# HengyiWang/spann3r

Measured on AMD Instinct MI355X. Metric: frames/sec/GPU (224px, 10-frame seq) + mem-bank cross-attn HBM GB/s, higher is better.
Workload: dtype bf16

## Files before the change

include/spann3r_hip.h:

```cpp
#ifndef SPANN3R_HIP_H
#define SPANN3R_HIP_H

#include <stdint.h>

#ifdef __cplusplus
extern "C" {
#endif

enum { SP3_F32 = 0, SP3_BF16 = 1 };
enum { SP3_ACT_NONE = 0, SP3_ACT_GELU = 1, SP3_ACT_RELU = 2 };
enum { SP3_EPI_PLAIN = 0, SP3_EPI_ROPE_VT = 1, SP3_EPI_PIXSHUF = 2, SP3_EPI_PARTIAL = 3 };
enum { SP3_LOAD_PLAIN = 0, SP3_LOAD_CONV3X3 = 1, SP3_LOAD_SOFTMAX = 2 };

const char* sp3_last_error(void);
int sp3_version(void);

typedef struct sp3_gemm_desc {
  const float* A;
  const float* A2;
  const void* W;
  void* C;
  const float* bias;
  const float* res1;
  const float* res2;
  int32_t M, N, K;
  int32_t batch;
  int32_t K1;
  int64_t lda, lda2, ldw, ldc, ldr1, ldr2;
  int64_t strideA, strideW, strideC;
  float alpha;
  int32_t wdtype;
  int32_t act;
  int32_t out_bf16;
  int32_t relu_in;
  int32_t loader;
  int32_t conv_H, conv_W, conv_C, conv_OH, conv_OW, conv_stride;
  int32_t epi;
  const float* rope_cos;
  const float* rope_sin;
  const int32_t* pos;
  int32_t rope_cols;
  void* vt;
  int32_t tokens;
  int32_t heads;
  int64_t vt_ld;
  int32_t ps_k, ps_H, ps_W, ps_C;
  int32_t tile;
  int32_t a_bf16;
  int32_t splitk;
  int32_t a_packed;
  const float* ln_stats;
  const float* ln_s;
  int32_t ln_nt;
  int32_t ln_C;
  float ln_eps;
  float* stats_out;
  void* c2;
  int32_t qkv_packed;
  int32_t out_packed;
  int32_t w_packed;
  int64_t sb_A2, sb_bias, sb_ln_stats, sb_ln_s, sb_stats_out, sb_c2, sb_vt;
  int64_t* trace;
  float* sm_stats_out;
  const float* sm_stats;
  int32_t sm_nt;
  float sm_thresh;
  float* sm_zout;
  int32_t f32x3;
  int32_t res_bf16;
  const int32_t* dyn_n;
} sp3_gemm_desc;
int sp3_gemm(const sp3_gemm_desc* desc_host, void* stream);
int sp3_gemm2(const sp3_gemm_desc* a, const sp3_gemm_desc* b, void* stream);
int sp3_gemm_plan(const sp3_gemm_desc* desc_host);

int sp3_layernorm(const float* x, int64_t ldx, const float* gamma, const float* beta, float eps,
                  void* out, int64_t ldo, int out_bf16, int rows, int C, void* stream);
int sp3_layernorm_packed(const float* x, int64_t ldx, const float* gamma, const float* beta, float eps,
                         void* out, int out_bf16, int rows, int C, void* stream);
int sp3_layernorm_dual(const float* x, int64_t ldx, const float* gamma, const float* beta, float eps, float* out, int64_t ldo,
                       void* out_packed_bf16, int rows, int C, int group_rows, int group_rows_pad, void* stream);
int sp3_layernorm_t(const float* x, int64_t ldx, const float* gamma, const float* beta, float eps,
                    void* out, int64_t ldo, int out_bf16, int rows, int C, void* stream);

typedef struct sp3_reduce_ln_desc {
  const float* partial;
  int64_t split_stride;
  const float* bias;
  const float* res;
  int64_t ldres;
  float* x_out;
  int64_t ldx;
  const float* g1; const float* b1; void* out1; int64_t ld1; int32_t out1_bf16;
  const float* g2; const float* b2; void* out2; int64_t ld2; int32_t out2_bf16;
  float eps;
  int32_t splits, rows, C;
  int32_t out1_packed, out2_packed;
  int32_t act;
  const float* res2;
  int64_t ldres2;
} sp3_reduce_ln_desc;
int sp3_reduce_ln(const sp3_reduce_ln_desc* desc_host, void* stream);

int sp3_rope_2d(void* tokens, int dtype, int B, int N, int H, int D, int64_t sB, int64_t sN, int64_t sH,
                const int64_t* positions, float base, float fwd, void* stream);

int sp3_attention(const void* q, int64_t sq, int64_t ldq, const void* k, int64_t sk, int64_t ldk,
                  const void* vt, int64_t vt_ld, void* out, int64_t ldo, int out_bf16,
                  int B, int heads, int Nq, int Nk, float scale, int dtype, void* stream);
int sp3_attention_ex(const void* q, int64_t sq, int64_t ldq, const void* k, int64_t sk, int64_t ldk,
                     const void* vt, int64_t vt_ld, void* out, int64_t ldo, int out_bf16, int out_packed,
                     int B, int heads, int Nq, int Nk, float scale, int dtype, void* stream);

int sp3_attention_packed(const void* qp, int q_cols, int q_col0, int npad_q, const void* kp, int k_cols, int k_col0, int npad_k,
                         const void* vtp, void* out, int64_t ldo, int out_bf16, int out_packed,
                         int B, int heads, int Nq, int Nk, float scale, int o_group, int o_group_rows, void* stream);

typedef struct sp3_attn_qproj_desc {
  const void* x_packed; int64_t x_group_stride;
  const float* ln_stats; int64_t stats_group_stride;
  const void* w_packed; int64_t w_group_stride;
  const float* ln_s; const float* bias; int64_t vec_group_stride;
  const int32_t* pos; const float* rope_cos; const float* rope_sin;
  float ln_eps; int32_t D;
  const void* kp; int32_t k_cols, k_col0, npad_k; const void* vtp;
  void* out; int64_t ldo; int32_t out_bf16, out_packed;
  int32_t B, heads, Nq, Nk; float scale; int32_t o_group, o_group_rows;
} sp3_attn_qproj_desc;
int sp3_attention_packed_qproj(const sp3_attn_qproj_desc* desc_host, void* stream);

typedef struct sp3_bank_write_desc {
  const float* feat_k;
  const float* feat_v;
  float* k_raw;
  float* v_raw;
  void* k_hat;
  void* v_hat_t;
  float* s_bank;
  float* b_bank;
  const float *gamma_k, *beta_k, *gamma_v, *beta_v, *gamma_q, *beta_q;
  float eps;
  float alpha;
  int32_t M, P, C, cap;
  int32_t wdtype;
  const int32_t* state;
} sp3_bank_write_desc;
int sp3_bank_write(const sp3_bank_write_desc* desc_host, void* stream);
int sp3_softmax_thresh(const float* S, float* P, int64_t ld, int64_t strideS, int rows, int M, int Mpad,
                       float thresh, int batch, void* P_packed, int64_t stride_packed, int packed_bf16, void* stream);
int sp3_softmax_pack(const float* S, int64_t ld, int64_t strideS, int rows, int M, float thresh, int batch, void* P_packed,
                     int64_t stride_packed, int packed_bf16, float* rowstat_ws, void* stream);
int sp3_colsum_accum(const float* P, int64_t ld, int rows, int M, float* mem_attn, void* stream);
int sp3_colsum_packed(const void* P_packed, int packed_bf16, int rows, int M, float* mem_attn, void* stream);
int sp3_colsum_softmax(const float* S, int64_t ld, int rows, int M, const float* rowz, float thresh, float* mem_attn,
                       float* mem_count, int append_P, void* stream);
int sp3_pack_stats(const float* x, int64_t ldx, int rows, int C, void* packed, int packed_bf16, float* stats, void* stream);
// ... 131 lines not shown
```

spann3r_amd/csrc/common.h:

```cpp
#pragma once
#include <hip/hip_runtime.h>
#include <stdint.h>
#include <stdio.h>
#include "../../include/spann3r_hip.h"

typedef __attribute__((ext_vector_type(8))) __bf16 bf16x8;
typedef __attribute__((ext_vector_type(4))) __bf16 bf16x4;
typedef __attribute__((ext_vector_type(2))) __bf16 bf16x2;
typedef __attribute__((ext_vector_type(4))) float f32x4;

#define SP3_WAVE 64

void sp3_set_error(const char* fmt, ...);

#define SP3_CHECK(cond, ...)                     \
  do {                                           \
    if (!(cond)) {                               \
      sp3_set_error(__VA_ARGS__);                \
      return 1;                                  \
    }                                            \
  } while (0)

#define SP3_LAUNCH_CHECK(what)                                              \
  do {                                                                      \
    hipError_t e_ = hipGetLastError();                                      \
    if (e_ != hipSuccess) {                                                 \
      sp3_set_error("%s: launch failed: %s", what, hipGetErrorString(e_));  \
      return 2;                                                             \
    }                                                                       \
  } while (0)

__device__ __forceinline__ float wave_sum(float v) {
#pragma unroll
  for (int o = 32; o > 0; o >>= 1) v += __shfl_xor(v, o);
  return v;
}
__device__ __forceinline__ float wave_max(float v) {
#pragma unroll
  for (int o = 32; o > 0; o >>= 1) v = fmaxf(v, __shfl_xor(v, o));
  return v;
}

__device__ __forceinline__ bf16x8 cvt8(const float4 a, const float4 b) {
  bf16x8 r;
  r[0] = (__bf16)a.x; r[1] = (__bf16)a.y; r[2] = (__bf16)a.z; r[3] = (__bf16)a.w;
  r[4] = (__bf16)b.x; r[5] = (__bf16)b.y; r[6] = (__bf16)b.z; r[7] = (__bf16)b.w;
  return r;
}

__device__ __forceinline__ float4 relu4(float4 v) {
  v.x = fmaxf(v.x, 0.f); v.y = fmaxf(v.y, 0.f); v.z = fmaxf(v.z, 0.f); v.w = fmaxf(v.w, 0.f);
  return v;
}

__device__ __forceinline__ float gelu_erf(float x) {
  const float a = fabsf(x);
  const float t = __builtin_amdgcn_rcpf(fmaf(0.2316419f, a, 1.0f));
  float p = fmaf(1.330274429f, t, -1.821255978f);
  p = fmaf(p, t, 1.781477937f);
  p = fmaf(p, t, -0.356563782f);
  p = fmaf(p, t, 0.319381530f);
  const float e = __builtin_amdgcn_exp2f(-0.72134752044448170368f * a * a);
  const float q = (p * t) * (e * 0.3989422804014327f);
  return fmaf(-a, q, fmaxf(x, 0.f));
}

#ifndef SP3_NO_WT_STORES
__device__ __forceinline__ void st_out(bf16x4* p, bf16x4 v) {
  __hip_atomic_store(reinterpret_cast<unsigned long long*>(p), __builtin_bit_cast(unsigned long long, v), __ATOMIC_RELAXED, __HIP_MEMORY_SCOPE_AGENT);
}
__device__ __forceinline__ void st_out(float2* p, float2 v) {
  __hip_atomic_store(reinterpret_cast<unsigned long long*>(p), __builtin_bit_cast(unsigned long long, v), __ATOMIC_RELAXED, __HIP_MEMORY_SCOPE_AGENT);
}
__device__ __forceinline__ void st_out(float4* p, float4 v) {
  const f32x4 t = {v.x, v.y, v.z, v.w};
  asm volatile("global_store_dwordx4 %0, %1, off sc1\n\ts_nop 1" ::"v"(p), "v"(t) : "memory");
}
__device__ __forceinline__ void st_out(bf16x8* p, bf16x8 v) {
  asm volatile("global_store_dwordx4 %0, %1, off sc1\n\ts_nop 1" ::"v"(p), "v"(v) : "memory");
}
#else
template <typename T> __device__ __forceinline__ void st_out(T* p, T v) { *p = v; }
#endif

__device__ __forceinline__ int64_t packed_off(int row, int k, int K, bool bf16) {
  const int lkb = bf16 ? 6 : 5, lch = bf16 ? 4 : 3;
  const int nkb = (K + (1 << lkb) - 1) >> lkb;
  const int kb = k >> lkb, kk = k & ((1 << lkb) - 1);
  const int g = kk >> lch, e = kk & ((1 << lch) - 1);
  const int h = e >> (lch - 1), eh = e & ((1 << (lch - 1)) - 1);
  return (((((int64_t)(row >> 4) * nkb + kb) * 2 + h) * 4 + g) * 16 + (row & 15)) * (1 << (lch - 1)) + eh;
}
```

spann3r_amd/csrc/gemm.hip:

```cpp
#include "common.h"
#include "gemm_sm.h"
#include <cstdlib>
#include <type_traits>

namespace {

struct GemmArgs {
  sp3_gemm_desc d;
  sp3_gemm_desc d2;
  int nb1;
  int xcd_slices;
};

template <typename TA, typename TW> struct MM;

__device__ __forceinline__ bf16x8 zero8() {
  bf16x8 z;
#pragma unroll
  for (int i = 0; i < 8; ++i) z[i] = (__bf16)0.f;
  return z;
}

__device__ __forceinline__ bf16x8 relu8(bf16x8 v) {
#pragma unroll
  for (int i = 0; i < 8; ++i) v[i] = (float)v[i] > 0.f ? v[i] : (__bf16)0.f;
  return v;
}

typedef __attribute__((ext_vector_type(4))) unsigned int u32x4;

__device__ __forceinline__ bf16x8 mask8(bf16x8 v, unsigned m) {
  u32x4 b = __builtin_bit_cast(u32x4, v);
  b &= m;
  return __builtin_bit_cast(bf16x8, b);
}
__device__ __forceinline__ float4 mask4(float4 v, unsigned m) {
  v.x = __uint_as_float(__float_as_uint(v.x) & m);
  v.y = __uint_as_float(__float_as_uint(v.y) & m);
  v.z = __uint_as_float(__float_as_uint(v.z) & m);
  v.w = __uint_as_float(__float_as_uint(v.w) & m);
  return v;
}

struct WRegB { bf16x8 v[2]; };
__device__ __forceinline__ void loadW_b(WRegB& r, const __bf16* p, int off1) {
  r.v[0] = *reinterpret_cast<const bf16x8*>(p);
  r.v[1] = *reinterpret_cast<const bf16x8*>(p + off1);
}
__device__ __forceinline__ void fixW_b(WRegB& r, unsigned m0, unsigned m1) {
  r.v[0] = mask8(r.v[0], m0);
  r.v[1] = mask8(r.v[1], m1);
}

template <> struct MM<float, __bf16> {
  static constexpr int KB = 64;
  static constexpr int CH = 16;
  struct AReg { float4 v[4]; };
  using WReg = WRegB;
  static __device__ __forceinline__ void loadA(AReg& r, const float* p, int off1) {
    const float4* q = reinterpret_cast<const float4*>(p);
    const float4* q1 = reinterpret_cast<const float4*>(p + off1);
    r.v[0] = q[0]; r.v[1] = q[1]; r.v[2] = q1[0]; r.v[3] = q1[1];
  }
  static __device__ __forceinline__ void fixA(AReg& r, unsigned m0, unsigned m1, bool relu) {
    r.v[0] = mask4(r.v[0], m0); r.v[1] = mask4(r.v[1], m0); r.v[2] = mask4(r.v[2], m1); r.v[3] = mask4(r.v[3], m1);
    if (relu) { r.v[0] = relu4(r.v[0]); r.v[1] = relu4(r.v[1]); r.v[2] = relu4(r.v[2]); r.v[3] = relu4(r.v[3]); }
  }
  static __device__ __forceinline__ void loadW(WReg& r, const __bf16* p, int off1) { loadW_b(r, p, off1); }
  static __device__ __forceinline__ void fixW(WReg& r, unsigned m0, unsigned m1) { fixW_b(r, m0, m1); }
  template <int MF, int NF>
  static __device__ __forceinline__ void mma(f32x4 (&acc)[MF][NF], const AReg (&a)[MF], const WReg (&w)[NF]) {
#pragma unroll
    for (int m = 0; m < MF; ++m) {
      const bf16x8 a0 = cvt8(a[m].v[0], a[m].v[1]);
      const bf16x8 a1 = cvt8(a[m].v[2], a[m].v[3]);
#pragma unroll
      for (int n = 0; n < NF; ++n) {
        acc[m][n] = __builtin_amdgcn_mfma_f32_16x16x32_bf16(a0, w[n].v[0], acc[m][n], 0, 0, 0);
        acc[m][n] = __builtin_amdgcn_mfma_f32_16x16x32_bf16(a1, w[n].v[1], acc[m][n], 0, 0, 0);
      }
    }
  }
  template <int MF, int NF>
  static __device__ __forceinline__ void mma_half(f32x4 (&)[MF][NF], const AReg (&)[MF], const WReg (&)[NF]) {}
};

template <> struct MM<__bf16, __bf16> {
  static constexpr int KB = 64;
  static constexpr int CH = 16;
  struct AReg { bf16x8 v[2]; };
  using WReg = WRegB;
  static __device__ __forceinline__ void loadA(AReg& r, const __bf16* p, int off1) {
    r.v[0] = *reinterpret_cast<const bf16x8*>(p);
// ... 220 lines not shown
  const TA* base[MF];
  __device__ __forceinline__ void init(const sp3_gemm_desc& d, const TA* A, int row0, int lane, int, int) {
#pragma unroll
    for (int m = 0; m < MF; ++m) {
      int r = row0 + m * 16 + (lane & 15);
      r = r < d.M ? r : d.M - 1;
      base[m] = A + (int64_t)r * d.lda;
    }
  }
  __device__ __forceinline__ const TA* ptr(const sp3_gemm_desc&, int m, int k, int, int, bool& inb) const {
    inb = true;
    return base[m] + k;
  }
};

__device__ __forceinline__ float4 smx4(float4 s, float c, float thr, int left, float& z) {
  constexpr float L2E = 1.44269504088896341f;
  float p[4] = {__builtin_amdgcn_exp2f(fmaf(s.x, L2E, c)), __builtin_amdgcn_exp2f(fmaf(s.y, L2E, c)),
                __builtin_amdgcn_exp2f(fmaf(s.z, L2E, c)), __builtin_amdgcn_exp2f(fmaf(s.w, L2E, c))};
#pragma unroll
  for (int e = 0; e < 4; ++e) {
    p[e] = (p[e] < thr || e >= left) ? 0.f : p[e];
    z += p[e];
  }
  return make_float4(p[0], p[1], p[2], p[3]);
}

template <typename TA, int MF> struct ARows<TA, SP3_LOAD_CONV3X3, MF> {
  const TA* img[MF];
  int iy0[MF], ix0[MF];
  const TA* safe;
  __device__ __forceinline__ void init(const sp3_gemm_desc& d, const TA* A, int row0, int lane, int, int) {
    safe = A;
#pragma unroll
    for (int m = 0; m < MF; ++m) {
      int r = row0 + m * 16 + (lane & 15);
      r = r < d.M ? r : d.M - 1;
      const int per = d.conv_OH * d.conv_OW;
      const int b = r / per;
      const int rem = r - b * per;
      const int oy = rem / d.conv_OW;
      const int ox = rem - oy * d.conv_OW;
      img[m] = A + (int64_t)b * d.conv_H * d.conv_W * d.conv_C;
      iy0[m] = oy * d.conv_stride - 1;
      ix0[m] = ox * d.conv_stride - 1;
    }
  }
  __device__ __forceinline__ const TA* ptr(const sp3_gemm_desc& d, int m, int k, int, int, bool& inb) const {
    const int tap = k / d.conv_C;
    const int ci = k - tap * d.conv_C;
    const int dy = tap / 3;
    const int iy = iy0[m] + dy;
    const int ix = ix0[m] + (tap - dy * 3);
    inb = (iy >= 0) && (iy < d.conv_H) && (ix >= 0) && (ix < d.conv_W);
    return inb ? img[m] + ((int64_t)iy * d.conv_W + ix) * d.conv_C + ci : safe;
  }
};

__device__ __forceinline__ void glds16(const char* gsrc, char* lds) {
#if defined(__HIP_DEVICE_COMPILE__)
  __builtin_amdgcn_global_load_lds((const __attribute__((address_space(1))) void*)gsrc,
                                   (__attribute__((address_space(3))) void*)lds, 16, 0, 0);
#else
  (void)gsrc; (void)lds;
#endif
}

template <typename TA, int LOADER, int MF, int NF, int WK>
constexpr int gemm_min_waves() { return (sizeof(TA) == 2 && LOADER == SP3_LOAD_PLAIN && MF == 2 && NF == 2 && WK == 4) ? 3 : 1; }

template <int I, int N, typename F>
__device__ __forceinline__ void static_for(F&& f) {
  if constexpr (I < N) {
    if (f(std::integral_constant<int, I>{})) static_for<I + 1, N>(f);
  }
}

constexpr int kWRing = 12;
constexpr int kMaxKb = 64;

template <typename TA, typename TW, int LOADER, int MF, int NF, int WM, int WN, int WK, int STAGES, int LOOP = 0, int XM = 0>
__global__ __launch_bounds__(64 * (WM * WN * WK + (LOOP >= 2 ? LOOP : 0)), (gemm_min_waves<TA, LOADER, MF, NF, WK>()))
void gemm_kernel(const GemmArgs args) {
  const bool second = args.nb1 > 0 && (int)blockIdx.y >= args.nb1;
  sp3_gemm_desc d = second ? args.d2 : args.d;
  using M_ = MM<TA, TW>;
  constexpr bool LDSK = LOOP != 0;
  constexpr int NCW = WM * WN * WK;
  constexpr int BM = MF * 16 * WM, BN = NF * 16 * WN, NT = 64 * (NCW + (LOOP >= 2 ? LOOP : 0));
  constexpr int KB = M_::KB, CH = M_::CH;
  constexpr int LDS_LD = BN + 4;
  extern __shared__ __attribute__((aligned(16))) float smem[];

  const int mt = (d.M + BM - 1) / BM, nt = (d.N + BN - 1) / BN;
  int tile_m, tile_n;
  int bx = blockIdx.x, kz = blockIdx.z;
  if (args.xcd_slices) {
    const unsigned L = blockIdx.x + gridDim.x * blockIdx.z, xc = L & 7, jj = L >> 3, q = jj / gridDim.x;
    kz = (int)(xc + 8 * q);
    bx = (int)(jj - q * gridDim.x);
  }
  {
    const int b = bx, xcd = b & 7, j = b >> 3;
    if (mt >= nt) {
      tile_n = j % nt;
      tile_m = (j / nt) * 8 + xcd;
    } else {
      tile_m = j % mt;
      tile_n = (j / mt) * 8 + xcd;
    }
  }
  if (tile_m >= mt || tile_n >= nt) return;

  const int tid = threadIdx.x, lane = tid & 63, wave = tid >> 6;
  const int wk = wave % WK, wn = (wave / WK) % WN, wm = wave / (WK * WN);
  const int g = lane >> 4;
  const int bz = second ? (int)blockIdx.y - args.nb1 : (int)blockIdx.y;
  if (d.batch > 1) {
    auto shift = [&](auto*& p, int64_t bytes) {
      using P = std::remove_reference_t<decltype(p)>;
      if (p) p = reinterpret_cast<P>(reinterpret_cast<uintptr_t>(p) + (uintptr_t)(bz * bytes));
    };
    shift(d.A2, d.sb_A2); shift(d.bias, d.sb_bias); shift(d.ln_stats, d.sb_ln_stats); shift(d.ln_s, d.sb_ln_s);
    shift(d.stats_out, d.sb_stats_out); shift(d.c2, d.sb_c2); shift(d.vt, d.sb_vt);
    const int64_t csz = d.epi == SP3_EPI_ROPE_VT ? (int64_t)sizeof(TW) : (d.out_bf16 ? 2 : 4);
    shift(d.C, d.strideC * csz);
    d.strideC = 0;
  }
  const TA* A = reinterpret_cast<const TA*>(d.A) + (int64_t)bz * d.strideA;
  const TW* W = reinterpret_cast<const TW*>(d.W) + (int64_t)bz * d.strideW;

  const int m0 = tile_m * BM, n0 = tile_n * BN;
  int64_t* tr0 = ((LOOP == 0 || LOOP == -1) && args.d.trace && blockIdx.x < 8 && blockIdx.y == 0 && blockIdx.z == 0 && threadIdx.x == 0) ? args.d.trace + blockIdx.x * 64 : nullptr;
  if (tr0) { tr0[0] = clock64(); tr0[3] = wall_clock64(); }
  ARows<TA, LOADER, MF> arows;
  arows.init(d, A, m0 + wm * MF * 16, lane, M_::KB, M_::CH);
  const TW* wbase[NF];
  int64_t wstep;
  if (d.w_packed) {
    const int nkb_pad = (int)((d.ldw + KB - 1) / KB);
    wstep = 64 * CH;
#pragma unroll
    for (int n = 0; n < NF; ++n) {
      int nb = (n0 + wn * NF * 16 + n * 16) >> 4;
      const int nb_max = (d.N + 15) / 16 - 1;
      nb = nb < nb_max ? nb : nb_max;
      wbase[n] = W + ((int64_t)nb * nkb_pad * 128 + lane) * (CH / 2);
    }
  } else {
    wstep = KB;
#pragma unroll
    for (int n = 0; n < NF; ++n) {
      int c = n0 + wn * NF * 16 + n * 16 + (lane & 15);
      c = c < d.N ? c : d.N - 1;
      wbase[n] = W + (int64_t)c * d.ldw + g * CH;
    }
  }

  f32x4 acc[MF][NF];
  constexpr bool XACC = sizeof(TA) == 4 && sizeof(TW) == 4 && (XM == 4 || XM == 5);
  f32x4 accx[XACC ? MF : 1][XACC ? NF : 1];
#pragma unroll
  for (int m = 0; m < MF; ++m)
#pragma unroll
    for (int n = 0; n < NF; ++n) acc[m][n] = f32x4{0.f, 0.f, 0.f, 0.f};
  if constexpr (XACC) {
#pragma unroll
    for (int m = 0; m < MF; ++m)
#pragma unroll
      for (int n = 0; n < NF; ++n) accx[m][n] = f32x4{0.f, 0.f, 0.f, 0.f};
  }

  static_assert(NT % (BN / 4) == 0, "epilogue column group must be fixed per thread");
  const int ec4 = (tid % (BN / 4)) * 4;
  const bool epre = (n0 + ec4 + 4) <= d.N && (d.N & 3) == 0 && d.epi != SP3_EPI_PIXSHUF;
  float4 pre_b4 = make_float4(0.f, 0.f, 0.f, 0.f), pre_s4 = pre_b4;
  if (epre) {
    if (d.bias) pre_b4 = *reinterpret_cast<const float4*>(d.bias + n0 + ec4);
    if (d.ln_stats) pre_s4 = *reinterpret_cast<const float4*>(d.ln_s + n0 + ec4);
  }

  constexpr int TPR = NT >= 8 * BM ? 8 : NT >= 4 * BM ? 4 : NT >= 2 * BM ? 2 : 1;
  constexpr int NPRE = (LDSK && LOOP != -1 && STAGES >= 3) ? 32 / TPR : 4;
  const int srow = tid / TPR, sj = tid % TPR;
  float2 sp[NPRE];
#pragma unroll
  for (int q = 0; q < NPRE; ++q) sp[q] = make_float2(0.f, 0.f);
  const float2* sps = nullptr;
  constexpr bool LNF = LOADER == SP3_LOAD_PLAIN && LOOP < 2;
  if (LNF && d.ln_stats && srow < BM) {
    const int sgm = (m0 + srow) < d.M ? (m0 + srow) : d.M - 1;
    sps = reinterpret_cast<const float2*>(d.ln_stats) + (int64_t)sgm * d.ln_nt;
#pragma unroll
    for (int q = 0; q < NPRE; ++q) {
      const int t = sj + q * TPR;
      sp[q] = sps[t < d.ln_nt ? t : d.ln_nt - 1];
    }
  }

  const int nkb_all = (d.K + KB - 1) / KB;
  const int per = (nkb_all + d.splitk - 1) / d.splitk;
  const int kb_lo = kz * per;
  const int kb_hi = (kb_lo + per) < nkb_all ? (kb_lo + per) : nkb_all;
  const bool relu = d.relu_in != 0;

  typename M_::AReg a[STAGES][MF];
  typename M_::WReg w[STAGES][NF];
  unsigned am0[STAGES][MF], am1[STAGES][MF], wm0[STAGES], wm1[STAGES];
  constexpr bool CONV = LOADER == SP3_LOAD_CONV3X3;
  constexpr bool SMX = LOADER == SP3_LOAD_SOFTMAX;
  float sm_c[MF], sm_z[MF];
  int sm_left[STAGES];
#pragma unroll
  for (int m = 0; m < MF; ++m) { sm_c[m] = 0.f; sm_z[m] = 0.f; }

  auto load = [&](auto full_tag, int st, int kb) {
// ... 853 lines not shown
      off = (((int64_t)b * d.ps_H * d.ps_k + y * d.ps_k + ky) * ((int64_t)d.ps_W * d.ps_k) + x * d.ps_k + kx) * d.ps_C + co;
    } else if (d.out_packed) {
      off = packed_off(gm, gn, d.N, d.out_bf16 != 0);
    } else {
      off = (int64_t)bz * d.strideC + (int64_t)gm * d.ldc + gn;
    }
    if (pre_res && idx == tid) {
      v[0] += pre_r1.x + pre_r2.x; v[1] += pre_r1.y + pre_r2.y; v[2] += pre_r1.z + pre_r2.z; v[3] += pre_r1.w + pre_r2.w;
    } else {
      if (d.res1) {
        const float* r = d.res1 + ((int64_t)bz * d.M + gm) * d.ldr1 + gn;
#pragma unroll
        for (int e = 0; e < 4; ++e) if (e < nvalid) v[e] += r[e];
      }
      if (d.res2) {
        const float* r = d.res2 + ((int64_t)bz * d.M + gm) * d.ldr2 + gn;
#pragma unroll
        for (int e = 0; e < 4; ++e) if (e < nvalid) v[e] += r[e];
      }
    }
    if (d.sm_stats_out) {
      float mx = -INFINITY;
#pragma unroll
      for (int e = 0; e < 4; ++e) if (e < nvalid) mx = fmaxf(mx, v[e]);
#pragma unroll
      for (int o_ = 1; o_ < 8; o_ <<= 1) mx = fmaxf(mx, __shfl_xor(mx, o_));
      float se = 0.f;
#pragma unroll
      for (int e = 0; e < 4; ++e) if (e < nvalid) se += __expf(v[e] - mx);
#pragma unroll
      for (int o_ = 1; o_ < 8; o_ <<= 1) se += __shfl_xor(se, o_);
      if (((gn >> 2) & 7) == 0)
        reinterpret_cast<float2*>(d.sm_stats_out)[(int64_t)gm * ((d.N + 31) >> 5) + (gn >> 5)] = make_float2(mx, se);
      if (nvalid <= 0) continue;
    }
    if (d.stats_out) {
      float s1 = (v[0] + v[1]) + (v[2] + v[3]);
      float s2 = (v[0] * v[0] + v[1] * v[1]) + (v[2] * v[2] + v[3] * v[3]);
#pragma unroll
      for (int o_ = 1; o_ < 8; o_ <<= 1) { s1 += __shfl_xor(s1, o_); s2 += __shfl_xor(s2, o_); }
      if (((gn >> 2) & 7) == 0)
        reinterpret_cast<float2*>(d.stats_out)[(int64_t)gm * (d.N >> 5) + (gn >> 5)] = make_float2(s1, s2);
    }
    if (d.c2) {
      const bool cb = d.wdtype == SP3_BF16;
      const int64_t o2 = packed_off(gm, gn, d.N, cb);
      if (cb) {
        bf16x4 ob;
        ob[0] = (__bf16)v[0]; ob[1] = (__bf16)v[1]; ob[2] = (__bf16)v[2]; ob[3] = (__bf16)v[3];
        *reinterpret_cast<bf16x4*>(reinterpret_cast<__bf16*>(d.c2) + o2) = ob;
      } else {
        *reinterpret_cast<float4*>(reinterpret_cast<float*>(d.c2) + o2) = make_float4(v[0], v[1], v[2], v[3]);
      }
    }
    if (d.out_bf16) {
      __bf16* o = reinterpret_cast<__bf16*>(d.C) + off;
      if (nvalid == 4 && ((off & 3) == 0)) {
        bf16x4 ob;
        ob[0] = (__bf16)v[0]; ob[1] = (__bf16)v[1]; ob[2] = (__bf16)v[2]; ob[3] = (__bf16)v[3];
        *reinterpret_cast<bf16x4*>(o) = ob;
      } else {
#pragma unroll
        for (int e = 0; e < 4; ++e) if (e < nvalid) o[e] = (__bf16)v[e];
      }
    } else {
      float* o = reinterpret_cast<float*>(d.C) + off;
      if (nvalid == 4 && ((off & 3) == 0)) {
        *reinterpret_cast<float4*>(o) = make_float4(v[0], v[1], v[2], v[3]);
      } else {
#pragma unroll
        for (int e = 0; e < 4; ++e) if (e < nvalid) o[e] = v[e];
      }
    }
  }
  if constexpr (LOOP >= 2) {
    if (d.trace && blockIdx.x < 8 && blockIdx.y == 0 && blockIdx.z == 0 && tid == 0) {
      d.trace[blockIdx.x * 64 + 2] = clock64();
      d.trace[blockIdx.x * 64 + 4] = wall_clock64();
    }
  }
  if (tr0) { tr0[2] = clock64(); tr0[4] = wall_clock64(); }
}

thread_local const sp3_gemm_desc* g_pair = nullptr;

template <typename TA, typename TW, int LOADER, int MF, int NF, int WM, int WN, int WK, int STAGES, int LOOP = 0, int XM = 0>
int launch(const sp3_gemm_desc& d, hipStream_t stream) {
  constexpr bool LDSK = LOOP != 0;
  constexpr int BM = MF * 16 * WM, BN = NF * 16 * WN, NT = 64 * (WM * WN * WK + (LOOP >= 2 ? LOOP : 0));
  auto grid_x = [](const sp3_gemm_desc& q) {
    const int mt = (q.M + BM - 1) / BM, nt = (q.N + BN - 1) / BN;
    return mt >= nt ? ((mt + 7) / 8) * 8 * nt : ((nt + 7) / 8) * 8 * mt;
  };
  int blocks = grid_x(d);
  size_t lds = ((size_t)WK * BM * (BN + 4) + 2 * BM) * sizeof(float);
  if (LDSK) {
    const size_t stages = (size_t)STAGES * (BM / 16 + (LOOP >= 2 ? 0 : BN / 16)) * 2048;
    lds = lds > stages ? lds : stages;
  }
  auto kern = gemm_kernel<TA, TW, LOADER, MF, NF, WM, WN, WK, STAGES, LOOP, XM>;
  if (lds > 64 * 1024) {
    static bool raised = false;
    if (!raised) {
      hipError_t e = hipFuncSetAttribute(reinterpret_cast<const void*>(kern), hipFuncAttributeMaxDynamicSharedMemorySize, (int)lds);
      if (e != hipSuccess) { sp3_set_error("sp3_gemm: cannot raise dynamic LDS to %zu: %s", lds, hipGetErrorString(e)); return 2; }
      raised = true;
    }
  }
  GemmArgs a;
  a.d = d;
  a.nb1 = 0;
  int gy = d.batch;
  if (g_pair) {
    a.d2 = *g_pair;
    a.nb1 = d.batch;
    gy += g_pair->batch;
    const int b2 = grid_x(*g_pair);
    blocks = blocks > b2 ? blocks : b2;
  } else {
    a.d2 = d;
  }
  a.xcd_slices = (gy == 1 && d.splitk >= 8 && d.splitk % 8 == 0 && blocks % 8 == 0) ? 1 : 0;
  hipLaunchKernelGGL(kern, dim3(blocks, gy, d.splitk), dim3(NT), lds, stream, a);
  SP3_LAUNCH_CHECK("sp3_gemm");
  return 0;
}

template <typename TA, typename TW, int LOADER>
int dispatch_tile(const sp3_gemm_desc& d, int tile, hipStream_t stream) {
  if constexpr (sizeof(TA) == 4 && sizeof(TW) == 4) {
    const int xm = d.f32x3;
    if (xm >= 1 && xm <= 4 && tile >= 0 && tile <= 2) {
#define SP3_XM_TILES(XM_)                                                                         \
      switch (tile) {                                                                             \
        case 0: return launch<TA, TW, LOADER, 2, 2, 1, 1, 4, 3, 0, XM_>(d, stream);               \
        case 1: return launch<TA, TW, LOADER, 2, 2, 2, 2, 1, 2, 0, XM_>(d, stream);               \
        default: return launch<TA, TW, LOADER, 2, 4, 2, 2, 1, 2, 0, XM_>(d, stream);              \
      }
      if (xm == 1) { SP3_XM_TILES(1) }
      if (xm == 2) { SP3_XM_TILES(2) }
      if (xm == 4 && d.w_packed == 2) { SP3_XM_TILES(5) }
      if (xm == 4) { SP3_XM_TILES(4) }
      SP3_XM_TILES(3)
#undef SP3_XM_TILES
    }
  }
  switch (tile) {
    case 0: return launch<TA, TW, LOADER, 2, 2, 1, 1, 4, 3>(d, stream);
    case 1: return launch<TA, TW, LOADER, 2, 2, 2, 2, 1, 2>(d, stream);
    case 2: return launch<TA, TW, LOADER, 2, 4, 2, 2, 1, 2>(d, stream);
    case 3: return launch<TA, TW, LOADER, 4, 4, 1, 1, 4, 3>(d, stream);
    case 4: case 18:
      if constexpr (sizeof(TA) == 2 && LOADER == SP3_LOAD_PLAIN) {
        if (tile == 4) return launch<TA, TW, LOADER, 2, 4, 1, 1, 4, 3>(d, stream);
        return launch<TA, TW, LOADER, 1, 4, 1, 1, 4, 3>(d, stream);
      }
      sp3_set_error("sp3_gemm: tile %d needs bf16 A and the plain loader", tile);
      return 1;
    case 20: case 21: case 22: case 23: case 24: case 25:
      if constexpr (sizeof(TA) == sizeof(TW) && LOADER == SP3_LOAD_PLAIN) {
        if (d.a_packed && d.w_packed && !d.A2 && d.K % MM<TA, TW>::KB == 0) {
          switch (tile) {
            case 20: return launch<TA, TW, LOADER, 4, 4, 4, 2, 1, 3, -1>(d, stream);
            case 21: return launch<TA, TW, LOADER, 4, 4, 2, 2, 2, 4, -1>(d, stream);
            case 22: return launch<TA, TW, LOADER, 4, 4, 2, 1, 2, 3, -1>(d, stream);
            case 24: return launch<TA, TW, LOADER, 4, 2, 1, 1, 2, 4, -1>(d, stream);
            case 25: return launch<TA, TW, LOADER, 2, 2, 1, 1, 2, 4, -1>(d, stream);
            default: return launch<TA, TW, LOADER, 4, 4, 1, 1, 2, 4, -1>(d, stream);
          }
        }
      }
      sp3_set_error("sp3_gemm: tile %d (pipelined LDS) needs fragment-order A and W in the MFMA dtype, whole k-blocks, no split A", tile);
      return 1;
    case 5: case 6: case 7: case 8: case 9: case 10: case 11: case 12: case 13: case 14: case 15: case 16: case 17:
      if constexpr (sizeof(TA) == sizeof(TW) && LOADER == SP3_LOAD_PLAIN) {
        if (d.a_packed && d.w_packed && !d.A2 && d.K % MM<TA, TW>::KB == 0) {
          switch (tile) {
            case 5: return launch<TA, TW, LOADER, 4, 4, 2, 2, 1, 2, 1>(d, stream);
            case 6: return launch<TA, TW, LOADER, 4, 2, 2, 2, 1, 2, 1>(d, stream);
            case 7: return launch<TA, TW, LOADER, 7, 1, 1, 4, 1, 4, 1>(d, stream);
            case 8: return launch<TA, TW, LOADER, 13, 1, 1, 4, 1, 3, 1>(d, stream);
            case 9: return launch<TA, TW, LOADER, 7, 1, 1, 2, 1, 4, 1>(d, stream);
            case 10: return launch<TA, TW, LOADER, 7, 2, 1, 2, 1, 4, 1>(d, stream);
            case 11: return launch<TA, TW, LOADER, 7, 1, 1, 4, 2, 4, 1>(d, stream);
            case 12: return launch<TA, TW, LOADER, 13, 1, 1, 4, 2, 3, 1>(d, stream);
            default: break;
          }
          const int nkb_slice = ((d.K / MM<TA, TW>::KB) + d.splitk - 1) / d.splitk;
          if (d.ln_stats && d.ln_nt > 32) {
            sp3_set_error("sp3_gemm: tile %d folds a LayerNorm over at most 1024 columns (ln_C=%d)", tile, d.ln_C);
            return 1;
          }
          if (nkb_slice > kMaxKb) {
            sp3_set_error("sp3_gemm: tile %d streams at most %d k-blocks per K slice (K=%d, splitk=%d)", tile, kMaxKb, d.K, d.splitk);
            return 1;
          }
          if constexpr (sizeof(TA) == 2) switch (tile) {
            case 13: return launch<TA, TW, LOADER, 7, 1, 1, 4, 2, 4, 2>(d, stream);
            case 14: return launch<TA, TW, LOADER, 7, 1, 1, 4, 1, 4, 2>(d, stream);
            case 15: return launch<TA, TW, LOADER, 13, 1, 1, 4, 2, 3, 2>(d, stream);
            case 16: return launch<TA, TW, LOADER, 7, 1, 1, 4, 1, 4, 6>(d, stream);
            case 17: return launch<TA, TW, LOADER, 7, 1, 1, 4, 2, 4, 4>(d, stream);
          }
// ... 67 lines not shown
    SP3_CHECK(d.rope_cols == 0 || (d.rope_cos && d.rope_sin && d.pos), "sp3_gemm: ROPE_VT needs tables and positions");
    SP3_CHECK(d.rope_cols == d.N || (d.vt && d.tokens > 0 && d.heads > 0 && d.vt_ld >= d.tokens), "sp3_gemm: ROPE_VT needs vt/tokens/heads");
    SP3_CHECK(!d.qkv_packed || (d.wdtype == SP3_BF16 && d.tokens > 0 && d.vt_ld % 64 == 0 && d.vt_ld >= d.tokens),
              "sp3_gemm: qkv_packed needs bf16, tokens and vt_ld (padded tokens per image, multiple of 64)");
  } else if (d.epi == SP3_EPI_PIXSHUF) {
    SP3_CHECK(d.ps_k > 0 && d.ps_C > 0 && d.ps_C % 4 == 0 && d.N == d.ps_k * d.ps_k * d.ps_C && d.M % (d.ps_H * d.ps_W) == 0,
              "sp3_gemm: bad PIXSHUF geometry");
  } else if (d.epi == SP3_EPI_PARTIAL) {
    SP3_CHECK(d.batch == 1 && d.ldc % 4 == 0 && d.ldc >= d.N, "sp3_gemm: PARTIAL needs batch 1 and ldc %% 4 == 0");
  } else {
    SP3_CHECK(d.epi == SP3_EPI_PLAIN, "sp3_gemm: bad epilogue %d", d.epi);
  }
  int tile = d.tile;
  if (tile < 0) {
    const long sk = d.splitk;
    const long t64 = (long)((d.M + 63) / 64) * ((d.N + 63) / 64) * d.batch * sk;
    const long t128 = (long)((d.M + 63) / 64) * ((d.N + 127) / 128) * d.batch;
    const bool lds_ok = d.loader == SP3_LOAD_PLAIN && !d.sm_stats_out && sk == 1 && d.a_packed && d.w_packed && d.a_bf16 && !d.A2 &&
                        d.epi != SP3_EPI_PARTIAL && d.K % 64 == 0;
    constexpr bool pipe_on = true;
    const bool pipe_ok = d.loader == SP3_LOAD_PLAIN && !d.sm_stats_out && d.a_packed && d.w_packed && d.a_bf16 && !d.A2 && d.K % 64 == 0 &&
                         (sk == 1 || d.epi == SP3_EPI_PARTIAL);
    const bool wide_legacy = lds_ok && d.M >= 1024 && d.N >= 2304 && d.N % 128 == 0 && d.N < 16384;
    if (pipe_ok && pipe_on && d.M >= 512 && d.epi != SP3_EPI_ROPE_VT && !wide_legacy) {
      const long mt256 = (d.M + 255) / 256, mt128 = (d.M + 127) / 128, nt128 = (d.N + 127) / 128, nt64 = (d.N + 63) / 64;
      if (mt256 * nt128 * d.batch * sk >= 144) tile = 20;
      else if (mt128 * nt128 * d.batch * sk >= 200) tile = 21;
      else if (mt128 * nt64 * d.batch * sk <= 192) tile = 24;
      else tile = 22;
    } else if (lds_ok && d.M >= 1024 && d.N >= 2304 && d.N % 128 == 0) {
      tile = (d.N % 4096 == 0 || (long)((d.M + 127) / 128) * (d.N / 128) * d.batch >= 1024) ? 5 : 6;
    } else if (d.loader == SP3_LOAD_SOFTMAX) {
      tile = 0;
    } else if (d.loader != SP3_LOAD_CONV3X3 && d.M >= 1024) {
      tile = 1;
      if (d.wdtype == SP3_F32 && !d.a_bf16 && sk == 1 && d.epi != SP3_EPI_PARTIAL && d.N % 128 == 0 && t128 >= 512) tile = 2;
    } else if (lds_ok && d.M <= 224 && d.M > 112 && d.epi == SP3_EPI_PLAIN && d.N >= 3072 && d.K <= 1024 &&
               (!d.ln_stats || d.ln_nt <= 32)) {
      tile = 13;
    } else if (d.loader == SP3_LOAD_CONV3X3 || d.M > 2048) {
      if (t128 >= 1024 && d.N % 128 == 0) tile = 2;
      else if (t64 >= 512) tile = 1;
      else tile = 0;
    } else {
      tile = 0;
      (void)t64;
    }
  }
  SP3_CHECK(!d.sm_stats_out || tile <= 3 || tile >= 20, "sp3_gemm: sm_stats_out needs a register-ring tile (0-3) or a pipelined one (20-25)");
  tile_out = tile;
  return 0;
}

static int gemm_dispatch(const sp3_gemm_desc& d, int tile, hipStream_t stream) {
  if (d.loader == SP3_LOAD_SOFTMAX) {
    if (d.tile == 1) {
      if (d.wdtype == SP3_BF16) return launch<float, __bf16, SP3_LOAD_SOFTMAX, 2, 2, 1, 1, 4, 3>(d, stream);
      return launch<float, float, SP3_LOAD_SOFTMAX, 2, 2, 1, 1, 4, 3>(d, stream);
    }
    if (d.wdtype == SP3_BF16) return launch<float, __bf16, SP3_LOAD_SOFTMAX, 1, 4, 1, 1, 4, 3>(d, stream);
    return launch<float, float, SP3_LOAD_SOFTMAX, 1, 4, 1, 1, 4, 3>(d, stream);
  }
  if (d.wdtype == SP3_BF16) {
    if (d.a_bf16) {
      if (d.loader == SP3_LOAD_PLAIN) return dispatch_tile<__bf16, __bf16, SP3_LOAD_PLAIN>(d, tile, stream);
      return dispatch_tile<__bf16, __bf16, SP3_LOAD_CONV3X3>(d, tile, stream);
    }
    if (d.loader == SP3_LOAD_PLAIN) return dispatch_tile<float, __bf16, SP3_LOAD_PLAIN>(d, tile, stream);
    return dispatch_tile<float, __bf16, SP3_LOAD_CONV3X3>(d, tile, stream);
  } else {
    if (d.loader == SP3_LOAD_PLAIN) return dispatch_tile<float, float, SP3_LOAD_PLAIN>(d, tile, stream);
    return dispatch_tile<float, float, SP3_LOAD_CONV3X3>(d, tile, stream);
  }
}

extern "C" int sp3_gemm(const sp3_gemm_desc* dp, void* stream_) {
  SP3_CHECK(dp != nullptr, "sp3_gemm: null descriptor");
  sp3_gemm_desc d = *dp;
  int tile = -1;
  if (int rc = gemm_prepare(d, tile)) return rc;
  if (d.tile >= 30 || (d.tile < 0 && sp3_gemm_sm_tile(d) >= 0)) return sp3_gemm_sm_launch(d, nullptr, reinterpret_cast<hipStream_t>(stream_));
  SP3_CHECK(!(d.a_packed && d.A2), "sp3_gemm: a fragment-order A split along K runs on the lean instances only (no instance for M=%d N=%d K=%d)", d.M, d.N, d.K);
  SP3_CHECK(!(d.res_bf16 && (d.res1 || d.res2)), "sp3_gemm: bf16 residual maps are read by the lean small-map convolutions only (res_bf16 = out_bf16 = a_bf16; M=%d N=%d K=%d)", d.M, d.N, d.K);
  SP3_CHECK(!d.dyn_n, "sp3_gemm: a device-side extent (dyn_n) is served by the lean memory-read instances only (tiles 43 / 44; M=%d N=%d K=%d)", d.M, d.N, d.K);
  return gemm_dispatch(d, tile, reinterpret_cast<hipStream_t>(stream_));
}

extern "C" int sp3_gemm_plan(const sp3_gemm_desc* dp) {
  if (!dp) return -1;
  sp3_gemm_desc d = *dp;
  d.tile = -1;
  int tile = -1;
  if (gemm_prepare(d, tile)) return -1;
  const int lean = sp3_gemm_sm_tile(d);
  return lean >= 0 ? lean : tile;
}

extern "C" int sp3_gemm2(const sp3_gemm_desc* ap, const sp3_gemm_desc* bp, void* stream_) {
  SP3_CHECK(ap != nullptr && bp != nullptr, "sp3_gemm2: null descriptor");
  sp3_gemm_desc a = *ap, b = *bp;
  int ta = -1, tb = -1;
  {
    sp3_gemm_desc a0 = a, b0 = b;
    int t0 = -1, t1 = -1;
    const int want = a0.tile;
    a0.tile = b0.tile = -1;
    if (gemm_prepare(a0, t0) == 0 && gemm_prepare(b0, t1) == 0) {
      const int la = sp3_gemm_sm_tile(a0), lb = sp3_gemm_sm_tile(b0);
      if (la >= 30 && la == lb && sp3_gemm_sm_pairs(a0) && (want < 0 || want == la)) return sp3_gemm_sm_launch(a0, &b0, reinterpret_cast<hipStream_t>(stream_));
    }
    SP3_CHECK(want < 30, "sp3_gemm2: tile %d asks for a lean instance that does not take this pair", want);
  }
  if (int rc = gemm_prepare(a, ta)) return rc;
  if (b.tile < 0) b.tile = ta;
  if (int rc = gemm_prepare(b, tb)) return rc;
  SP3_CHECK(!(a.res_bf16 && (a.res1 || a.res2)) && !(b.res_bf16 && (b.res1 || b.res2)), "sp3_gemm2: bf16 residual maps are read by the lean small-map convolutions only");
  SP3_CHECK(ta == tb && a.wdtype == b.wdtype && a.a_bf16 == b.a_bf16 && a.loader == b.loader && a.loader != SP3_LOAD_SOFTMAX,
            "sp3_gemm2: both groups must use one kernel instance (tile %d / %d, same dtypes and loader)", ta, tb);
  SP3_CHECK(a.splitk == 1 && b.splitk == 1 && !a.trace && !b.trace && !a.dyn_n && !b.dyn_n, "sp3_gemm2: no split-K, no trace, no device-side extent");
  g_pair = &b;
  const int rc = gemm_dispatch(a, ta, reinterpret_cast<hipStream_t>(stream_));
  g_pair = nullptr;
  return rc;
}
```

spann3r_amd/csrc/gemm_sm.h:

```cpp
#pragma once
#include "common.h"

int sp3_gemm_sm_tile(const sp3_gemm_desc& d);
bool sp3_gemm_sm_pairs(const sp3_gemm_desc& d);
int sp3_gemm_sm_launch(const sp3_gemm_desc& d, const sp3_gemm_desc* pair, hipStream_t stream);
```

spann3r_amd/csrc/gemm_sm.hip:

```cpp
#include "common.h"
#include "gemm_sm.h"
#include <cstdlib>
#include <type_traits>

namespace {

enum { SM_PACKED = 0, SM_STREAM = 1, SM_ROPE = 2, SM_SCORE = 3, SM_PROB = 4 };

struct SmOp {
  const char* A; const char* A2; const char* W; char* C;
  const float* bias; const float* res1; const float* ln_stats; const float* ln_s;
  float* stats_out; char* c2; char* vt;
  long gA, gA2, gW, gC, gbias, gres, gstats, gs, gso, gc2, gvt;
  int N, ntz, ldc, rope_cols, act, nkb1;
  int nt;
  int ngrp, nzb;
  float alpha;
};

struct SmArgs {
  SmOp op[2];
  const float* cos; const float* sin; const int* pos;
  int M, rb_max, z1;
  int mblk;
// ... 1040 lines not shown
#pragma unroll
        for (int e = 0; e < 4; ++e) acc[m][n][e] = fmaf(sc[m], tmp[m][n][e], acc[m][n][e]);
  }
  asm volatile("s_waitcnt vmcnt(0)" ::: "memory");
#pragma unroll
  for (int m = 0; m < MF; ++m)
    if (grow[m] < a.M)
#pragma unroll
      for (int n = 0; n < NF; ++n)
        st_out(reinterpret_cast<float4*>(part + (long)grow[m] * a.ldc + cw0 + n * 16), make_float4(acc[m][n][0], acc[m][n][1], acc[m][n][2], acc[m][n][3]));
}

bool pvs_ok(const sp3_gemm_desc& d) {
  return d.loader == SP3_LOAD_SOFTMAX && d.wdtype == SP3_BF16 && d.w_packed && d.a_bf16 && d.a_packed && d.sm_stats && d.epi == SP3_EPI_PARTIAL &&
         !d.out_bf16 && !d.out_packed && !d.bias && !d.res1 && !d.res2 && d.act == SP3_ACT_NONE && d.alpha == 1.0f && d.batch <= 1 &&
         d.splitk >= 8 && d.splitk % 8 == 0 && !d.ln_stats && !d.stats_out && !d.c2 && !d.trace && !d.sm_stats_out && !d.A2 && d.N % 128 == 0 &&
         d.K % 4 == 0 && d.K >= 4 && d.M >= 1 && d.M < 65536 && d.ldw % 64 == 0 && d.ldw >= d.K && (d.ldc & 3) == 0 && d.ldc >= d.N;
}

int pvs_dispatch(const sp3_gemm_desc& d, hipStream_t stream) {
  PvsArgs a;
  a.A = reinterpret_cast<const char*>(d.A); a.W = reinterpret_cast<const char*>(d.W); a.scale = d.sm_stats; a.part = reinterpret_cast<float*>(d.C);
  a.M = d.M; a.N = d.N; a.Mk = d.K; a.nkbc = (int)(d.ldw / 64); a.S_k = d.splitk; a.ldc = (int)d.ldc;
  a.rows_pad = (long)((d.M + 255) & ~255);
  a.dyn = d.dyn_n;
  constexpr int WM = 4, WN = 2, NF = 4, NST = 3, BM = 256, BN = 128;
  constexpr size_t lds = (size_t)NST * ((BM / 16 + BN / 16) * 2048 + BM * 4);
  static_assert(lds <= 160 * 1024, "stage ring must fit the LDS");
  auto kern = pvs_kernel<WM, WN, NF, NST>;
  static bool raised = false;
  if (!raised) {
    hipError_t e = hipFuncSetAttribute(reinterpret_cast<const void*>(kern), hipFuncAttributeMaxDynamicSharedMemorySize, (int)lds);
    if (e != hipSuccess) { sp3_set_error("sp3_gemm (long-bank P.V): cannot raise dynamic LDS to %zu: %s", lds, hipGetErrorString(e)); return 2; }
    raised = true;
  }
  const int mt = (d.M + BM - 1) / BM, nt = d.N / BN;
  hipLaunchKernelGGL(kern, dim3(8, mt * nt, d.splitk / 8), dim3(64 * WM * WN), lds, stream, a);
  SP3_LAUNCH_CHECK("sp3_gemm (long-bank P.V)");
  return 0;
}

bool pv_ok(const sp3_gemm_desc& d) {
  return d.loader == SP3_LOAD_SOFTMAX && d.wdtype == SP3_BF16 && d.w_packed && !d.a_bf16 && !d.a_packed && d.sm_stats && d.epi == SP3_EPI_PLAIN &&
         !d.out_bf16 && !d.out_packed && !d.bias && !d.res2 && d.act == SP3_ACT_NONE && d.alpha == 1.0f && d.batch <= 1 && d.splitk <= 1 &&
         !d.ln_stats && !d.stats_out && !d.trace && !d.sm_stats_out && !d.A2 && d.N % 64 == 0 && d.K % 4 == 0 && d.K >= 4 &&
         d.sm_nt == (d.K + 31) / 32 && d.sm_nt <= 8 * 32 && d.M >= 1 && d.M < 65536 * 16 && d.ldw % 64 == 0 && d.ldw >= d.K && (d.lda & 3) == 0 &&
         d.lda >= ((d.K + 63) & ~63) && (d.ldc & 3) == 0 && d.ldc >= d.N && (!d.res1 || (d.ldr1 & 3) == 0) && (!d.c2 || d.N % 64 == 0);
}

template <int NF, int WK, int R>
int pv_launch(const PvArgs& a, int M, int N, hipStream_t stream) {
  constexpr size_t lds = ((size_t)WK * 16 * (NF * 16 + 4) + 16 * 4) * sizeof(float);
  static_assert(lds <= 160 * 1024, "partial tiles must fit the LDS");
  auto kern = pv_kernel<NF, WK, R>;
  if (lds > 64 * 1024) {
    static bool raised = false;
    if (!raised) {
      hipError_t e = hipFuncSetAttribute(reinterpret_cast<const void*>(kern), hipFuncAttributeMaxDynamicSharedMemorySize, (int)lds);
      if (e != hipSuccess) { sp3_set_error("sp3_gemm (lean, softmax P.V): cannot raise dynamic LDS to %zu: %s", lds, hipGetErrorString(e)); return 2; }
      raised = true;
    }
  }
  const int nt = N / (NF * 16);
  hipLaunchKernelGGL(kern, dim3(8, (M + 15) / 16, (nt + 7) / 8), dim3(64 * WK), lds, stream, a);
  SP3_LAUNCH_CHECK("sp3_gemm (lean, softmax P.V)");
  return 0;
}

int pv_dispatch(const sp3_gemm_desc& d, hipStream_t stream) {
  PvArgs a;
  a.S = reinterpret_cast<const float*>(d.A); a.stats = reinterpret_cast<const float2*>(d.sm_stats); a.W = reinterpret_cast<const char*>(d.W);
  a.out = reinterpret_cast<float*>(d.C); a.res = d.res1; a.c2 = reinterpret_cast<char*>(d.c2); a.zout = d.sm_zout;
  a.M = d.M; a.Mk = d.K; a.N = d.N; a.ld = (int)d.lda; a.ng = d.sm_nt; a.nkbw = (int)(d.ldw / 64); a.ldc = (int)d.ldc; a.ldr = (int)d.ldr1;
  a.thr = d.sm_thresh;
  a.dyn = d.dyn_n;
  return pv_launch<4, 8, 2>(a, d.M, d.N, stream);
}

struct ConvSmArgs {
  const void* x; const char* W; void* out;
  const float* bias; const void* res1; const void* res2;
  int M, N, H, Wd, Cin, OH, OW, stride, nkb, relu_in, act;
  unsigned cin_magic, per_magic, ow_magic;
};

typedef __attribute__((ext_vector_type(4))) unsigned int csm_u32x4;

template <typename TM> struct CsmA;
template <> struct CsmA<float> {
  float4 v[4];
  __device__ __forceinline__ void load(const void* p) {
    const float4* q = reinterpret_cast<const float4*>(p);
    v[0] = q[0]; v[1] = q[1]; v[2] = q[2]; v[3] = q[3];
  }
  __device__ __forceinline__ void halves(unsigned mask, bool relu, bf16x8& h0, bf16x8& h1) const {
    float4 t[4];
#pragma unroll
    for (int q = 0; q < 4; ++q) {
      t[q].x = __uint_as_float(__float_as_uint(v[q].x) & mask); t[q].y = __uint_as_float(__float_as_uint(v[q].y) & mask);
      t[q].z = __uint_as_float(__float_as_uint(v[q].z) & mask); t[q].w = __uint_as_float(__float_as_uint(v[q].w) & mask);
      if (relu) t[q] = relu4(t[q]);
    }
    h0 = cvt8(t[0], t[1]);
    h1 = cvt8(t[2], t[3]);
  }
};
template <> struct CsmA<__bf16> {
  bf16x8 v[2];
  __device__ __forceinline__ void load(const void* p) {
    const bf16x8* q = reinterpret_cast<const bf16x8*>(p);
    v[0] = q[0]; v[1] = q[1];
  }
  __device__ __forceinline__ void halves(unsigned mask, bool relu, bf16x8& h0, bf16x8& h1) const {
    csm_u32x4 a = __builtin_bit_cast(csm_u32x4, v[0]), b = __builtin_bit_cast(csm_u32x4, v[1]);
    a &= mask; b &= mask;
    h0 = __builtin_bit_cast(bf16x8, a);
    h1 = __builtin_bit_cast(bf16x8, b);
    if (relu) {
#pragma unroll
      for (int i = 0; i < 8; ++i) {
        h0[i] = (float)h0[i] > 0.f ? h0[i] : (__bf16)0.f;
        h1[i] = (float)h1[i] > 0.f ? h1[i] : (__bf16)0.f;
      }
    }
  }
};
__device__ __forceinline__ float4 csm_load4(const float* p) { return *reinterpret_cast<const float4*>(p); }
__device__ __forceinline__ float4 csm_load4(const __bf16* p) {
  const bf16x4 t = *reinterpret_cast<const bf16x4*>(p);
  return make_float4((float)t[0], (float)t[1], (float)t[2], (float)t[3]);
}
__device__ __forceinline__ void csm_store4(float* p, const float (&v)[4]) { st_out(reinterpret_cast<float4*>(p), make_float4(v[0], v[1], v[2], v[3])); }
__device__ __forceinline__ void csm_store4(__bf16* p, const float (&v)[4]) {
  bf16x4 t;
  t[0] = (__bf16)v[0]; t[1] = (__bf16)v[1]; t[2] = (__bf16)v[2]; t[3] = (__bf16)v[3];
  st_out(reinterpret_cast<bf16x4*>(p), t);
}

template <typename TM, int MF, int NF, int WK, int R>
__global__ __launch_bounds__(64 * WK) void conv_sm_kernel(const ConvSmArgs a) {
  constexpr int BM = MF * 16, BN = NF * 16, NT = 64 * WK, LD = BN + 4, CG = BN / 4;
  extern __shared__ __attribute__((aligned(16))) float smem[];
  const int tid = threadIdx.x, lane = tid & 63, wk = __builtin_amdgcn_readfirstlane(tid >> 6);
  const int tile_m = blockIdx.y, tile_n = blockIdx.z * 8 + blockIdx.x;
  const int m0 = tile_m * BM, n0 = tile_n * BN;
  if (n0 >= a.N) return;
  const int g = lane >> 4, r16 = lane & 15;
  const TM* X = reinterpret_cast<const TM*>(a.x);

  const int ec4 = (tid % CG) * 4, erow = tid / CG;
  const bool eact = erow < BM && (m0 + erow) < a.M;
  float4 b4 = make_float4(0.f, 0.f, 0.f, 0.f), r1 = b4, r2 = b4;
  if (eact) {
    const long o = (long)(m0 + erow) * a.N + n0 + ec4;
    if (a.bias) b4 = *reinterpret_cast<const float4*>(a.bias + n0 + ec4);
    if (a.res1) r1 = csm_load4(reinterpret_cast<const TM*>(a.res1) + o);
    if (a.res2) r2 = csm_load4(reinterpret_cast<const TM*>(a.res2) + o);
  }

  const TM* img[MF];
  int iy0[MF], ix0[MF];
#pragma unroll
  for (int m = 0; m < MF; ++m) {
    int r = m0 + m * 16 + r16;
    r = r < a.M ? r : a.M - 1;
    const int per = a.OH * a.OW;
    const int b = (int)__umulhi((unsigned)r, a.per_magic);
    const int rem = r - b * per;
    const int oy = (int)__umulhi((unsigned)rem, a.ow_magic), ox = rem - oy * a.OW;
    img[m] = X + (long)b * a.H * a.Wd * a.Cin;
    iy0[m] = oy * a.stride - 1;
    ix0[m] = ox * a.stride - 1;
  }
  const char* wp[NF];
#pragma unroll
  for (int n = 0; n < NF; ++n) wp[n] = a.W + ((long)(tile_n * NF + n) * a.nkb) * 2048 + lane * 16;

  CsmA<TM> av[R][MF];
  bf16x8 wv[R][NF][2];
  unsigned am[R][MF];
  auto load = [&](int slot, int kb) {
#pragma unroll
    for (int n = 0; n < NF; ++n) {
      wv[slot][n][0] = *reinterpret_cast<const bf16x8*>(wp[n] + (long)kb * 2048);
      wv[slot][n][1] = *reinterpret_cast<const bf16x8*>(wp[n] + (long)kb * 2048 + 1024);
    }
    const int k0 = kb * 64 + g * 16;
    const int tap = (int)__umulhi((unsigned)k0, a.cin_magic), ci = k0 - tap * a.Cin;
    const int dy = (tap * 11) >> 5, dx = tap - 3 * dy;
#pragma unroll
    for (int m = 0; m < MF; ++m) {
      const int iy = iy0[m] + dy, ix = ix0[m] + dx;
      const bool inb = iy >= 0 && iy < a.H && ix >= 0 && ix < a.Wd;
      am[slot][m] = inb ? 0xffffffffu : 0u;
      av[slot][m].load(inb ? img[m] + ((long)iy * a.Wd + ix) * a.Cin + ci : X);
    }
  };
  f32x4 acc[MF][NF];
#pragma unroll
  for (int m = 0; m < MF; ++m)
#pragma unroll
    for (int n = 0; n < NF; ++n) acc[m][n] = f32x4{0.f, 0.f, 0.f, 0.f};
  const int nkw = (a.nkb - wk + WK - 1) / WK;
#pragma unroll
  for (int i = 0; i < R; ++i)
    if (i < nkw) load(i, wk + i * WK);
  const bool relu = a.relu_in != 0;
  for (int i0 = 0; i0 < nkw; i0 += R) {
#pragma unroll
    for (int s = 0; s < R; ++s) {
      const int i = i0 + s;
      if (i < nkw) {
        bf16x8 ab[MF][2];
#pragma unroll
        for (int m = 0; m < MF; ++m) av[s][m].halves(am[s][m], relu, ab[m][0], ab[m][1]);
#pragma unroll
        for (int m = 0; m < MF; ++m)
#pragma unroll
          for (int n = 0; n < NF; ++n) {
            acc[m][n] = __builtin_amdgcn_mfma_f32_16x16x32_bf16(ab[m][0], wv[s][n][0], acc[m][n], 0, 0, 0);
            acc[m][n] = __builtin_amdgcn_mfma_f32_16x16x32_bf16(ab[m][1], wv[s][n][1], acc[m][n], 0, 0, 0);
          }
        if (i + R < nkw) load(s, wk + (i + R) * WK);
      }
    }
  }
  {
    float* slab = smem + (size_t)wk * BM * LD;
#pragma unroll
    for (int m = 0; m < MF; ++m)
#pragma unroll
      for (int n = 0; n < NF; ++n)
#pragma unroll
        for (int r = 0; r < 4; ++r) slab[(m * 16 + 4 * g + r) * LD + n * 16 + r16] = acc[m][n][r];
  }
  __syncthreads();
  static_assert(BM * CG <= NT, "one epilogue item per thread");
  if (eact) {
    float4 t = *reinterpret_cast<const float4*>(smem + erow * LD + ec4);
#pragma unroll
    for (int s = 1; s < WK; ++s) {
      const float4 u = *reinterpret_cast<const float4*>(smem + (size_t)s * BM * LD + erow * LD + ec4);
      t.x += u.x; t.y += u.y; t.z += u.z; t.w += u.w;
    }
    float v[4] = {t.x + b4.x, t.y + b4.y, t.z + b4.z, t.w + b4.w};
    if (a.act == SP3_ACT_RELU) {
#pragma unroll
      for (int e = 0; e < 4; ++e) v[e] = fmaxf(v[e], 0.f);
    }
    v[0] += r1.x + r2.x; v[1] += r1.y + r2.y; v[2] += r1.z + r2.z; v[3] += r1.w + r2.w;
    csm_store4(reinterpret_cast<TM*>(a.out) + (long)(m0 + erow) * a.N + n0 + ec4, v);
  }
}

template <typename TM, int MF, int NF, int WK, int R>
int conv_sm_launch(const ConvSmArgs& a, hipStream_t stream) {
  constexpr int BM = MF * 16, BN = NF * 16;
  constexpr size_t lds = (size_t)WK * BM * (BN + 4) * sizeof(float);
  static_assert(lds <= 64 * 1024, "partial tiles: default dynamic LDS limit");
  const int mt = (a.M + BM - 1) / BM, ntz = (a.N / BN + 7) / 8;
  hipLaunchKernelGGL((conv_sm_kernel<TM, MF, NF, WK, R>), dim3(8, mt, ntz), dim3(64 * WK), lds, stream, a);
  SP3_LAUNCH_CHECK("sp3_gemm (lean conv3x3)");
  return 0;
}

int conv_sm_tile(const sp3_gemm_desc& d) {
  if (d.loader != SP3_LOAD_CONV3X3 || d.wdtype != SP3_BF16 || !d.w_packed || (d.a_bf16 != 0) != (d.out_bf16 != 0) || d.out_packed || d.epi != SP3_EPI_PLAIN ||
      d.batch > 1 || d.splitk > 1 || d.alpha != 1.0f || d.ln_stats || d.stats_out || d.c2 || d.trace || d.sm_stats_out || d.f32x3)
    return -1;
  if (d.K % 64 || d.conv_C % 16 || d.K != 9 * d.conv_C || d.K >= 65536 || d.M > 2048 || d.M < 1 || d.act == SP3_ACT_GELU) return -1;
  if (d.ldc != d.N || (d.res1 && d.ldr1 != d.N) || (d.res2 && d.ldr2 != d.N) || (d.ldw > 0 && d.ldw != d.K)) return -1;
  if ((d.res1 || d.res2) && (d.res_bf16 != 0) != (d.out_bf16 != 0)) return -1;
  if (d.conv_OW < 2 || d.conv_OH * d.conv_OW < 2 || d.conv_C < 2) return -1;
  if (d.M <= 256) return d.N % 16 == 0 ? 40 : -1;
  return d.N % 32 == 0 ? 41 : -1;
}

int conv_sm_dispatch(const sp3_gemm_desc& d, int tile, hipStream_t stream) {
  ConvSmArgs a;
  a.x = d.A; a.W = reinterpret_cast<const char*>(d.W); a.out = d.C;
  a.bias = d.bias; a.res1 = d.res1; a.res2 = d.res2;
  a.M = d.M; a.N = d.N; a.H = d.conv_H; a.Wd = d.conv_W; a.Cin = d.conv_C; a.OH = d.conv_OH; a.OW = d.conv_OW;
  a.stride = d.conv_stride; a.nkb = d.K / 64; a.relu_in = d.relu_in; a.act = d.act;
  auto magic = [](int v) { return (unsigned)((1ull << 32) / (unsigned)v + 1); };
  a.cin_magic = magic(d.conv_C); a.per_magic = magic(d.conv_OH * d.conv_OW); a.ow_magic = magic(d.conv_OW);
  if (d.a_bf16) {
    if (tile == 40) return conv_sm_launch<__bf16, 1, 1, 12, 3>(a, stream);
    return conv_sm_launch<__bf16, 2, 2, 8, 3>(a, stream);
  }
  if (tile == 40) return conv_sm_launch<float, 1, 1, 12, 3>(a, stream);
  return conv_sm_launch<float, 2, 2, 8, 3>(a, stream);
}

struct SmInst {
  int tile, epi, K, MF, NF, WK;
  bool split;
  int min_n;
  int max_n;
  int (*launch)(const SmArgs&, int mt, int nz, hipStream_t);
  int min_m = 1, max_m = 256;
  int bm = 0, bn = 0;
  int min_mb = 0, max_mb = 1 << 30;
  int tile_m() const { return bm ? bm : MF * 16; }
  int tile_n() const { return bn ? bn : NF * 16; }
};

template <int MF, int NF, int WK, int NKB, int RING, int EPI, bool SPLIT = false>
int sm_launch(const SmArgs& a, int mt, int nz, hipStream_t stream) {
  constexpr int BM = MF * 16, BN = NF * 16;
  constexpr size_t lds = ((size_t)WK * BM * (BN + 4) + 2 * BM) * sizeof(float);
  static_assert(lds <= 160 * 1024, "partial tiles must fit the LDS");
  auto kern = sm_kernel<MF, NF, WK, NKB, RING, EPI, SPLIT>;
  if (lds > 64 * 1024) {
    static bool raised = false;
    if (!raised) {
      hipError_t e = hipFuncSetAttribute(reinterpret_cast<const void*>(kern), hipFuncAttributeMaxDynamicSharedMemorySize, (int)lds);
      if (e != hipSuccess) { sp3_set_error("sp3_gemm (lean): cannot raise dynamic LDS to %zu: %s", lds, hipGetErrorString(e)); return 2; }
      raised = true;
    }
  }
  hipLaunchKernelGGL(kern, dim3(8, mt, nz), dim3(64 * WK), lds, stream, a);
  SP3_LAUNCH_CHECK("sp3_gemm (lean)");
  return 0;
}

const SmInst kInst[] = {
    {30, SM_ROPE, 1024, 3, 4, 8, false, 0, 1 << 30, sm_launch<3, 4, 8, 16, 0, SM_ROPE>},
    {31, SM_ROPE, 768, 2, 2, 4, false, 0, 1 << 30, sm_launch<2, 2, 4, 12, 0, SM_ROPE>},
    {32, SM_PACKED, 1024, 4, 4, 8, false, 0, 1 << 30, sm_launch<4, 4, 8, 16, 0, SM_PACKED>},
    {33, SM_PACKED, 768, 2, 4, 4, false, 0, 1 << 30, sm_launch<2, 4, 4, 12, 0, SM_PACKED>},
    {42, SM_PACKED, 1792, 4, 2, 7, true, 0, 1 << 30, sm_launch<4, 2, 7, 28, 0, SM_PACKED, true>},
    {39, SM_STREAM, 1024, 3, 2, 8, false, 0, 768, sm_launch<3, 2, 8, 16, 0, SM_STREAM>},
    {34, SM_STREAM, 1024, 2, 2, 8, false, 769, 1 << 30, sm_launch<2, 2, 8, 16, 0, SM_STREAM>},
    {35, SM_STREAM, 4096, 2, 2, 8, false, 0, 1 << 30, sm_launch<2, 2, 8, 64, 4, SM_STREAM>},
    {36, SM_STREAM, 768, 3, 2, 6, false, 0, 1 << 30, sm_launch<3, 2, 6, 12, 0, SM_STREAM>},
    {37, SM_STREAM, 3072, 3, 2, 8, false, 0, 1 << 30, sm_launch<3, 2, 8, 48, 3, SM_STREAM>},
    {38, SM_STREAM, 1792, 4, 2, 7, false, 0, 1 << 30, sm_launch<4, 2, 7, 28, 0, SM_STREAM>},
    {43, SM_SCORE, 1024, 2, 2, 8, false, 0, 1 << 30, sm_launch<2, 2, 8, 16, 0, SM_SCORE>},
    {45, SM_PROB, 1024, 4, 4, 1, false, 0, 1 << 30, bm_launch<4, 2, 4, 16, 3, SM_PROB>, 257, 1 << 30, 256, 128},
    {50, SM_ROPE, 1024, 4, 4, 1, false, 0, 1 << 30, bm_launch<4, 2, 4, 16, 3, SM_ROPE>, 1536, 1 << 30, 256, 128},
    {51, SM_ROPE, 1024, 4, 4, 1, false, 0, 1 << 30, bm_launch<2, 2, 4, 16, 3, SM_ROPE>, 257, 1535, 128, 128},
    {52, SM_ROPE, 768, 4, 4, 1, false, 0, 1 << 30, bm_launch<2, 2, 4, 12, 3, SM_ROPE>, 257, 1 << 30, 128, 128, 0, 2047},
    {63, SM_ROPE, 768, 4, 4, 1, false, 1536, 1 << 30, bm_launch<4, 2, 4, 12, 3, SM_ROPE>, 257, 1 << 30, 256, 128, 2048, 1 << 30},
    {65, SM_ROPE, 768, 4, 2, 1, false, 0, 1535, bm_launch<2, 2, 2, 12, 3, SM_ROPE>, 257, 1 << 30, 128, 64, 2048, 1 << 30},
    {53, SM_PACKED, 1024, 4, 4, 1, false, 0, 1 << 30, bm_launch<4, 2, 4, 16, 3, SM_PACKED>, 1536, 1 << 30, 256, 128},
    {54, SM_PACKED, 1024, 4, 4, 1, false, 0, 1 << 30, bm_launch<2, 2, 4, 16, 3, SM_PACKED>, 257, 1535, 128, 128},
    {55, SM_PACKED, 768, 4, 4, 1, false, 0, 1 << 30, bm_launch<2, 2, 4, 12, 3, SM_PACKED>, 257, 1 << 30, 128, 128, 0, 2047},
    {64, SM_PACKED, 768, 4, 4, 1, false, 0, 1 << 30, bm_launch<4, 2, 4, 12, 3, SM_PACKED>, 257, 1 << 30, 256, 128, 2048, 1 << 30},
    {61, SM_STREAM, 1024, 4, 4, 1, false, 0, 1 << 30, bm_launch<4, 2, 4, 16, 3, SM_STREAM>, 4096, 1 << 30, 256, 128},
    {62, SM_STREAM, 4096, 4, 4, 1, false, 0, 1 << 30, bm_launch<4, 2, 4, 64, 3, SM_STREAM>, 4096, 1 << 30, 256, 128},
    {66, SM_PACKED, 1792, 4, 4, 1, true, 0, 1 << 30, bm_launch<2, 2, 4, 28, 3, SM_PACKED, true>, 257, 1 << 30, 128, 128, 0, 2047},
    {67, SM_PACKED, 1792, 4, 4, 1, true, 0, 1 << 30, bm_launch<4, 2, 4, 28, 3, SM_PACKED, true>, 257, 1 << 30, 256, 128, 2048, 1 << 30},
    {56, SM_STREAM, 1024, 4, 2, 1, false, 0, 1 << 30, bm_launch<2, 2, 2, 16, 3, SM_STREAM>, 257, 1 << 30, 128, 64},
    {57, SM_STREAM, 4096, 4, 2, 1, false, 0, 1 << 30, bm_launch<2, 2, 2, 64, 3, SM_STREAM>, 257, 1 << 30, 128, 64},
    {58, SM_STREAM, 768, 4, 2, 1, false, 0, 1 << 30, bm_launch<2, 2, 2, 12, 3, SM_STREAM>, 257, 1 << 30, 128, 64},
    {59, SM_STREAM, 3072, 4, 2, 1, false, 0, 1 << 30, bm_launch<2, 2, 2, 48, 4, SM_STREAM>, 257, 1 << 30, 128, 64},
    {60, SM_STREAM, 1792, 4, 2, 1, false, 0, 1 << 30, bm_launch<2, 2, 2, 28, 3, SM_STREAM>, 257, 1 << 30, 128, 64},
};
bool sm_enabled() {
  static const bool on = [] { const char* e = getenv("SP3_LEAN_GEMM"); return !(e && e[0] == '0'); }();
  return on;
}

int sm_kind(const sp3_gemm_desc& d) {
  if (d.sm_stats_out) return (d.out_packed && d.out_bf16) ? SM_PROB : SM_SCORE;
  if (d.epi == SP3_EPI_ROPE_VT) return SM_ROPE;
  if (d.out_packed) return SM_PACKED;
  return SM_STREAM;
}

const SmInst* sm_find(const sp3_gemm_desc& d) {
  if (!sm_enabled()) return nullptr;
  if (d.wdtype != SP3_BF16 || !d.a_bf16 || !d.a_packed || !d.w_packed || d.loader != SP3_LOAD_PLAIN || d.res2 || d.relu_in ||
      d.trace || d.sm_stats || (d.alpha != 1.0f && !d.sm_stats_out) || d.f32x3)
    return nullptr;
  if (d.splitk > 1 || d.epi == SP3_EPI_PARTIAL || d.epi == SP3_EPI_PIXSHUF) return nullptr;
  if (d.batch > 2 || d.M < 1 || d.M >= 65536 || (d.ldw > 0 && d.ldw != d.K) || !d.bias) return nullptr;
  const int kind = sm_kind(d);
  if (d.dyn_n && kind != SM_SCORE && kind != SM_PROB) return nullptr;
  if (kind == SM_PROB) {
    if (d.epi != SP3_EPI_PLAIN || d.batch > 1 || d.res1 || d.stats_out || d.c2 || d.act != SP3_ACT_NONE || d.N % 4 || d.N < 4 ||
        d.ldc % 64 || d.ldc < d.N || !d.ln_stats)
      return nullptr;
  } else
  if (kind == SM_SCORE) {
    if (d.epi != SP3_EPI_PLAIN || d.out_bf16 || d.out_packed || d.batch > 1 || d.res1 || d.stats_out || d.c2 || d.act != SP3_ACT_NONE ||
        d.N % 4 || d.N < 4 || (d.ldc & 3) || d.ldc < d.N || d.M > 256)
      return nullptr;
  } else if (kind == SM_ROPE) {
    if (!d.qkv_packed || d.rope_cols % 64 || d.N % 64 || (d.tokens & 3) || d.tokens <= 0 || d.tokens >= 65536 || d.vt_ld % 64) return nullptr;
    if (d.rope_cols < d.N && !d.vt) return nullptr;
  } else if (kind == SM_PACKED) {
    if (!d.out_bf16 || d.res1 || d.stats_out || d.c2 || d.act == SP3_ACT_RELU) return nullptr;
  } else {
    if (d.out_bf16 || d.out_packed || d.act != SP3_ACT_NONE || (d.ldc & 3) || d.ldc < d.N) return nullptr;
    if (d.res1 && d.ldr1 != d.N) return nullptr;
    if ((d.stats_out || d.c2) && d.N % 32) return nullptr;
  }
  if (d.ln_stats && (d.ln_C != d.K || d.K > 1024 || (d.K / 64) % 4)) return nullptr;
  const bool split = d.A2 != nullptr;
  if (split && (d.K1 % 64 || d.K1 <= 0 || d.K1 >= d.K)) return nullptr;
  for (const SmInst& s : kInst) {
    if (s.epi != kind || s.K != d.K || s.split != split || d.M < s.min_m || d.M > s.max_m) continue;
    const long mb = (long)d.M * (d.batch > 1 ? d.batch : 1);
    if (mb < s.min_mb || mb > s.max_mb) continue;
    if ((kind != SM_SCORE && kind != SM_PROB && d.N % s.tile_n()) || d.N < s.min_n || d.N > s.max_n) continue;
    if (!s.bm && d.ln_stats && s.MF * 16 * 4 > 64 * s.WK) continue;
    if (s.bm && kind == SM_ROPE && d.rope_cols % 32) continue;
    return &s;
  }
  return nullptr;
}

void sm_fill(SmOp& o, const sp3_gemm_desc& d, const SmInst& s) {
  const long G = d.batch > 1 ? 1 : 0;
  o.A = reinterpret_cast<const char*>(d.A);
  o.A2 = d.A2 ? reinterpret_cast<const char*>(d.A2) : o.A;
  o.nkb1 = d.A2 ? d.K1 / 64 : d.K / 64;
  o.gA2 = G * d.sb_A2;
  o.W = reinterpret_cast<const char*>(d.W);
  o.C = reinterpret_cast<char*>(d.C);
  o.bias = d.bias; o.res1 = d.res1; o.ln_stats = d.ln_stats; o.ln_s = d.ln_s;
  o.stats_out = d.stats_out; o.c2 = reinterpret_cast<char*>(d.c2); o.vt = reinterpret_cast<char*>(d.vt);
  o.gA = G * d.strideA * 2; o.gW = G * d.strideW * 2;
  o.gC = G * d.strideC * (s.epi == SM_STREAM ? 4 : 2);
  o.gbias = G * d.sb_bias; o.gres = G * (long)d.M * d.ldr1 * 4; o.gstats = G * d.sb_ln_stats; o.gs = G * d.sb_ln_s;
  o.gso = G * d.sb_stats_out; o.gc2 = G * d.sb_c2; o.gvt = G * d.sb_vt;
  o.N = d.N;
  o.alpha = d.alpha;
  if (s.epi == SM_SCORE || s.epi == SM_PROB) o.stats_out = d.sm_stats_out;
  o.nt = (d.N + s.tile_n() - 1) / s.tile_n();
  o.ntz = (o.nt + 7) / 8;
  o.ngrp = d.batch > 1 ? d.batch : 1;
  o.nzb = (o.ngrp * o.nt + 7) / 8;
  o.ldc = (int)d.ldc;
  o.rope_cols = d.rope_cols;
  o.act = d.act;
}

}

int sp3_gemm_sm_tile(const sp3_gemm_desc& d) {
  if (d.loader == SP3_LOAD_CONV3X3) return sm_enabled() ? conv_sm_tile(d) : -1;
  if (d.loader == SP3_LOAD_SOFTMAX) return !sm_enabled() ? -1 : pv_ok(d) ? 44 : pvs_ok(d) ? 46 : -1;
  const SmInst* s = sm_find(d);
  return s ? s->tile : -1;
}

bool sp3_gemm_sm_pairs(const sp3_gemm_desc& d) {
  if (d.loader != SP3_LOAD_PLAIN) return false;
  const SmInst* s = sm_find(d);
  return s && s->epi == SM_ROPE;
}

int sp3_gemm_sm_launch(const sp3_gemm_desc& d, const sp3_gemm_desc* pair, hipStream_t stream) {
  if (d.loader == SP3_LOAD_SOFTMAX && sm_enabled() && pvs_ok(d) && !pair && (d.tile < 30 || d.tile == 46)) return pvs_dispatch(d, stream);
  if (d.loader == SP3_LOAD_SOFTMAX) {
    if (!sm_enabled() || !pv_ok(d) || pair || (d.tile >= 30 && d.tile != 44)) {
      sp3_set_error("sp3_gemm: no lean softmax-loader instance for this descriptor (tile %d, M=%d N=%d K=%d)", d.tile, d.M, d.N, d.K);
      return 1;
    }
    return pv_dispatch(d, stream);
  }
  if (d.loader == SP3_LOAD_CONV3X3) {
    const int t = sm_enabled() ? conv_sm_tile(d) : -1;
    if (t < 0 || pair || (d.tile >= 30 && d.tile != t)) {
      sp3_set_error("sp3_gemm: no lean conv3x3 instance for this descriptor (tile %d, M=%d N=%d K=%d)", d.tile, d.M, d.N, d.K);
      return 1;
    }
    return conv_sm_dispatch(d, t, stream);
  }
  const SmInst* s = sm_find(d);
  if (!s || (d.tile >= 30 && d.tile != s->tile)) {
    sp3_set_error("sp3_gemm: no lean small-M instance for this descriptor (tile %d, M=%d N=%d K=%d epi=%d)", d.tile, d.M, d.N, d.K, d.epi);
    return 1;
  }
  SmArgs a;
  sm_fill(a.op[0], d, *s);
  a.op[1] = a.op[0];
  const int G0 = d.batch > 1 ? d.batch : 1;
  int nz = s->bm ? a.op[0].nzb : a.op[0].ntz * G0;
  a.z1 = nz;
  if (pair) {
    const SmInst* s2 = sm_find(*pair);
    if (s2 != s || pair->M != d.M || pair->tokens != d.tokens || pair->heads != d.heads || pair->vt_ld != d.vt_ld || pair->pos != d.pos ||
        pair->rope_cos != d.rope_cos || pair->rope_sin != d.rope_sin || pair->ln_eps != d.ln_eps || s->epi != SM_ROPE) {
      sp3_set_error("sp3_gemm2: the two groups do not share a lean instance");
      return 1;
    }
    sm_fill(a.op[1], *pair, *s);
    nz += s->bm ? a.op[1].nzb : a.op[1].ntz * (pair->batch > 1 ? pair->batch : 1);
  }
  a.cos = d.rope_cos; a.sin = d.rope_sin; a.pos = d.pos;
  a.M = d.M;
  a.xm = (s->bm && !pair && d.M > d.N) ? 1 : 0;
  if (a.xm) {
    a.z1 = 1 << 30;
    const int NT = a.op[0].nt * a.op[0].ngrp, mt_ = (d.M + s->tile_m() - 1) / s->tile_m(), nzm = (mt_ + 7) / 8;
    if (NT % 8 == 0 && NT > 8 && nzm % 4 == 0) a.xm = 2;
  }
  a.mblk = 0;
  if (s->bm && !a.xm && !pair) {
    const int mt_ = (d.M + s->tile_m() - 1) / s->tile_m();
    if (mt_ >= 16 && mt_ % 8 == 0 && nz >= 2 && nz <= 4) a.mblk = 1;
  }
  a.rb_max = (d.M + 15) / 16 - 1;
  a.tokens = d.tokens > 0 ? d.tokens : 1;
  a.heads = d.heads;
  a.vt_ld = (int)d.vt_ld;
  a.tok_magic = (unsigned)((1ull << 32) / (unsigned)a.tokens + 1);
  a.ln_eps = d.ln_eps;
  a.dyn = d.dyn_n;
  const int mt = (d.M + s->tile_m() - 1) / s->tile_m();
  return s->launch(a, mt, nz, stream);
}
```

spann3r_amd/engine.py:

```python
import math
import os

import torch

from . import ops
from .lib import ACT_NONE, ACT_GELU, ACT_RELU
from .config import Spann3RConfig


def _rope_tables(max_pos, base, device):
    half = 32
    inv_freq = 1.0 / (base ** (torch.arange(0, half, 2).float() / half))
    t = torch.arange(max_pos, dtype=torch.float32)
    ang = torch.einsum("i,j->ij", t, inv_freq)
    return ang.cos().contiguous().to(device), ang.sin().contiguous().to(device)


def _rope_tables_narrow(max_pos, base, head_dim, device):
    D = head_dim // 2
    nf = D // 2
    assert nf <= 16 and head_dim % 4 == 0
    inv_freq = 1.0 / (base ** (torch.arange(0, D, 2).float() / D))
    t = torch.arange(max_pos, dtype=torch.float32)
    ang = torch.einsum("i,j->ij", t, inv_freq)
# ... 474 lines not shown
            upd(ao, D, "proj", xi, stq, xq)
            if self.fuse_cross_q and P < 512 and D == 768 and ops.LEAN:
                ops.attention_packed_qproj(xq, stq, w[g + "cq.w"], w[g + "cq.s"], w[g + "cq.b"], pos, self.cos, self.sin, ckp, D, 0, npad, cvtp,
                                           ao, D, B=2 * B, heads=Hh, Nq=P, Nk=P, scale=64 ** -0.5, o_group=B, o_group_rows=Rp, eps=1e-6,
                                           stats_group_stride=sb_st // 4, vec_group_stride=D)
            else:
                ops.proj_rope_vt(xq, w[g + "cq.w"], w[g + "cq.b"], cqp, 0, None, npad, M=R, N=D, K=D, lda=D, rope_cols=D,
                                 ln=ops.LnFold(stq, D, w[g + "cq.s"], 1e-6, sb_stats=sb_st, sb_s=D * 4),
                                 strideA=xq.stride, strideW=w[g + "cq.w"].stride, strideC=B * npad * D, sb={"bias": D * 4}, **rope)
                ops.attention_packed(cqp, D, 0, npad, ckp, D, 0, npad, cvtp, ao, D, B=2 * B, heads=Hh, Nq=P, Nk=P,
                                     scale=64 ** -0.5, o_group=B, o_group_rows=Rp)
            upd(ao, D, "cproj", xo, stq, xq)
            Hd = D * cfg.mlp_ratio
            ops.gemm(xq, w[g + "fc1.w"], h, M=R, N=Hd, K=D, lda=D, ldc=Hd, bias=w[g + "fc1.b"], act=ACT_GELU,
                     ln=ops.LnFold(stq, D, w[g + "fc1.s"], 1e-6, sb_stats=sb_st, sb_s=Hd * 4),
                     batch=2, strideA=xq.stride, strideW=w[g + "fc1.w"].stride, strideC=h.stride, sb={"bias": Hd * 4})
            if last:
                upd(h, Hd, "fc2", xo, None, None)
            else:
                upd(h, Hd, "fc2", xo, st[nx], xp[nx])
        normed = self.ws("decg_normed", (2, R, D))
        ops.layernorm(x[depth], w["dec_norm.w"], w["dec_norm.b"], 1e-6, normed, rows=2 * R, C_=D,
                      dual=self.wspg("decg_normed_packed", R, D) if self.adt == torch.bfloat16 else None, group_rows=R)
        outs = {}
        for s_ in (0, 1):
            outs[s_] = [(f1, f2)[s_]] + [x[l][s_].view(B, P, D) for l in range(1, depth)] + [normed[s_].view(B, P, D)]
        return outs[0], outs[1]

    def key_aux(self, R):
        E = self.cfg.enc_dim
        return self.wspg("keyg_packed", R, E), self.ws("keyg_stats", (2, R, E // 32, 2))

    def encode_feat_keys_grouped(self, feat1, feat2, normed1, normed2, R, out1, out2, feat1p=None, feat2p=None):
        self.activate()
        cfg, w = self.cfg, self.w
        E, D, Kd = cfg.enc_dim, cfg.dec_dim, cfg.key_dim
        dF, dN, dO = feat2.data_ptr() - feat1.data_ptr(), normed2.data_ptr() - normed1.data_ptr(), out2.data_ptr() - out1.data_ptr()
        assert dF % 16 == 0 and dN % 16 == 0 and dO % 16 == 0
        es = 2 if self.adt == torch.bfloat16 else 4
        h = self.wspg("keyg_hidden", R, Kd)
        packed = None
        if feat1p is not None and feat2p is not None and self.adt == torch.bfloat16 and ops.LEAN:
            np_ = self.wspg("decg_normed_packed", R, D)
            dFp = feat2p.data_ptr() - feat1p.data_ptr()
            assert dFp % 16 == 0
            packed = dict(A2=np_, lda2=D, K1=E, batch=2, strideA=dFp // 2, strideW=w["keyg.0.w"].stride, strideC=h.stride,
                          sb={"bias": Kd * 4, "A2": np_.stride * 2})
            ok = self._splitA_plan.get(R)
            if ok is None:
                ok = self._splitA_plan[R] = ops.gemm(feat1p, w["keyg.0.w"], h, M=R, N=Kd, K=Kd, lda=E, ldc=Kd, bias=w["keyg.0.b"],
                                                     act=ACT_GELU, plan_only=True, **packed) >= 30
            if not ok:
                packed = None
        if packed is not None:
            ops.gemm(feat1p, w["keyg.0.w"], h, M=R, N=Kd, K=Kd, lda=E, ldc=Kd, bias=w["keyg.0.b"], act=ACT_GELU, **packed)
        else:
            ops.gemm(feat1, w["keyg.0.w"], h, M=R, N=Kd, K=Kd, lda=E, ldc=Kd, bias=w["keyg.0.b"], act=ACT_GELU, A2=normed1, lda2=D, K1=E,
                     batch=2, strideA=dF // 4, strideW=w["keyg.0.w"].stride, strideC=h.stride, sb={"bias": Kd * 4, "A2": dN})
        kp, kst = self.key_aux(R)
        ops.gemm(h, w["keyg.2.w"], out1, M=R, N=E, K=Kd, lda=Kd, ldc=E, bias=w["keyg.2.b"], stats_out=kst, c2=kp,
                 batch=2, strideA=h.stride, strideW=w["keyg.2.w"].stride, strideC=dO // 4,
                 sb={"bias": E * 4, "stats_out": R * (E // 32) * 8, "c2": kp.stride * es})
        return kp.at(1), kst[1]

    def encode_feat_key(self, feat, dec_last, R, num, out, aux=False):
        self.activate()
        cfg, w = self.cfg, self.w
        E, D, Kd = cfg.enc_dim, cfg.dec_dim, cfg.key_dim
        h = self.wsp("key_hidden%d" % num, R, Kd)
        pre = "key%d." % num
        ops.gemm(feat, w[pre + "0.w"], h, M=R, N=Kd, K=Kd, lda=E, ldc=Kd, bias=w[pre + "0.b"], act=ACT_GELU,
                 A2=dec_last, lda2=D, K1=E)
        if aux:
            kp, kst = self.key_aux(R)
            ops.gemm(h, w[pre + "2.w"], out, M=R, N=E, K=Kd, lda=Kd, ldc=E, bias=w[pre + "2.b"], stats_out=kst[num - 1],
                     c2=kp.at(num - 1))
            return kp.at(num - 1), kst[num - 1]
        ops.gemm(h, w[pre + "2.w"], out, M=R, N=E, K=Kd, lda=Kd, ldc=E, bias=w[pre + "2.b"])
        return out

    def _conv_ws(self, head):
        return self.ws("conv_splitk_ws" + str(head), (1 << 23,))

    def _rcu(self, x, pre, B, H, W_, out, extra_res=None, tag=""):
        w, F = self.w, self.cfg.dpt_feat
        t = self.ws("rcu_tmp" + tag, (B * H * W_, F), self.mdt)
        sk = self._conv_ws(tag[:1])
        ops.conv3x3(x, w[pre + "c1.w"], t, B=B, H=H, W_=W_, Cin=F, Cout=F, bias=w[pre + "c1.b"], relu_in=True, act=ACT_RELU,
                    splitk_ws=sk)
        ops.conv3x3(t, w[pre + "c2.w"], out, B=B, H=H, W_=W_, Cin=F, Cout=F, bias=w[pre + "c2.b"], res1=x, res2=extra_res,
                    splitk_ws=sk)
        return out

    def _fusion(self, pre, B, H, W_, x0, x1, tag, crop=None):
        w, F = self.w, self.cfg.dpt_feat
        M = B * H * W_
        cur = x0
        if x1 is not None:
            s = self.ws("fus_sum_" + tag, (M, F), self.mdt)
            self._rcu(x1, pre + "u1", B, H, W_, s, extra_res=x0, tag=tag)
            cur = s
        r = self.ws("fus_rcu2_" + tag, (M, F), self.mdt)
        self._rcu(cur, pre + "u2", B, H, W_, r, tag=tag)
        oc = self.ws("fus_oc_" + tag, (M, F), self.mdt)
        ops.gemm(r, w[pre + "out.w"], oc, M=M, N=F, K=F, lda=F, ldc=F, bias=w[pre + "out.b"])
        OH, OW = (2 * H, 2 * W_) if crop is None else crop
        up = self.ws("fus_up_" + tag, (B * OH * OW, F), self.mdt)
        ops.upsample2x(oc, up, B=B, H=H, W_=W_, C_=F, outH=OH, outW=OW)
        return up, OH, OW

    def dpt_head(self, dec, B, nh, nw, num, want_raw=False):
        self.activate()
        cfg, w = self.cfg, self.w
        F, Lc = cfg.dpt_feat, cfg.dpt_last
        pre = "dpt%d." % num
        R = B * nh * nw
        hk = cfg.hooks
        dims = (cfg.enc_dim, cfg.dec_dim, cfg.dec_dim, cfg.dec_dim)
        ld = (96, 192, 384, 768)
        mdt = self.mdt
        t = [self.ws("dpt%d_pp%d" % (num, i), (R, ld[i]), mdt) for i in range(4)]
        pairable = len({dec[hk[i]].dtype for i in range(4)}) == 1
        import contextlib
        pair = ops.pair if pairable else contextlib.nullcontext
        for i0 in (0, 2):
            with pair():
                for i in (i0, i0 + 1):
                    ops.gemm(dec[hk[i]], w[pre + "pp%d.w" % i], t[i], M=R, N=ld[i], K=dims[i], lda=dims[i], ldc=ld[i], bias=w[pre + "pp%d.b" % i])
        c0 = 128 if self.wdt == torch.bfloat16 else ld[0]
        l0 = self.ws("dpt%d_l0" % num, (B * 16 * nh * nw, c0), mdt)
        l1 = self.ws("dpt%d_l1" % num, (B * 4 * nh * nw, ld[1]), mdt)
        with pair():
            ops.conv_transpose_ks(t[0], w[pre + "pp0t.w"], l0, B=B, H=nh, W_=nw, Cin=ld[0], Cout=c0, ks=4, bias=w[pre + "pp0t.b"])
            ops.conv_transpose_ks(t[1], w[pre + "pp1t.w"], l1, B=B, H=nh, W_=nw, Cin=ld[1], Cout=ld[1], ks=2, bias=w[pre + "pp1t.b"])
        l2 = t[2]
        h3, w3 = (nh - 1) // 2 + 1, (nw - 1) // 2 + 1
        l3 = self.ws("dpt%d_l3" % num, (B * h3 * w3, ld[3]), mdt)
        sk = self._conv_ws(num)
        ops.conv3x3(t[3], w[pre + "pp3c.w"], l3, B=B, H=nh, W_=nw, Cin=ld[3], Cout=ld[3], stride=2, bias=w[pre + "pp3c.b"],
                    splitk_ws=sk)
        geo = ((4 * nh, 4 * nw), (2 * nh, 2 * nw), (nh, nw), (h3, w3))
        rn = []
        for i, src in enumerate((l0, l1, l2, l3)):
            Hh, Ww = geo[i]
            o = self.ws("dpt%d_rn%d" % (num, i), (B * Hh * Ww, F), mdt)
            ops.conv3x3(src, w[pre + "rn%d.w" % i], o, B=B, H=Hh, W_=Ww, Cin=(c0 if i == 0 else ld[i]), Cout=F, splitk_ws=sk)
            rn.append(o)
        p4, H4, W4 = self._fusion(pre + "ref4.", B, h3, w3, rn[3], None, "%d_4" % num, crop=(nh, nw))
        p3, H3, W3 = self._fusion(pre + "ref3.", B, H4, W4, p4, rn[2], "%d_3" % num)
        p2, H2, W2 = self._fusion(pre + "ref2.", B, H3, W3, p3, rn[1], "%d_2" % num)
        p1, H1, W1 = self._fusion(pre + "ref1.", B, H2, W2, p2, rn[0], "%d_1" % num)
        a = self.ws("dpt%d_h0" % num, (B * H1 * W1, Lc), mdt)
        ops.conv3x3(p1, w[pre + "h0.w"], a, B=B, H=H1, W_=W1, Cin=F, Cout=Lc, bias=w[pre + "h0.b"])
        OH, OW = 2 * H1, 2 * W1
        u = self.ws("dpt%d_h0up" % num, (B * OH * OW, Lc), mdt)
        ops.upsample2x(a, u, B=B, H=H1, W_=W1, C_=Lc)
        c = self.ws("dpt%d_h2" % num, (B * OH * OW, Lc), mdt)
        ops.conv3x3(u, w[pre + "h2.w"], c, B=B, H=OH, W_=OW, Cin=Lc, Cout=Lc, bias=w[pre + "h2.b"], act=ACT_RELU)
        pts = self.ws("dpt_pts%d" % num, (B, OH, OW, 3))
        conf = self.ws("dpt_conf%d" % num, (B, OH, OW))
        raw = self.ws("dpt_raw%d" % num, (B, OH, OW, 4)) if want_raw else None
        ops.head_final(c, w[pre + "h4.w"], w[pre + "h4.b"], B * OH * OW, Lc, pts, conf, raw)
        return pts, conf, raw

    def encode_cur_value_feat(self, tok, out, res, pos32=None):
        self.activate()
        cfg, w = self.cfg, self.w
        B, P, Cv = tok.shape
        assert Cv == cfg.val_dim
        R, E = B * P, cfg.enc_dim
        zero_pos = self.ws("valf_zero_pos", (R, 2), torch.int32, zero=True)
        rope_tab = None
        if cfg.mem_pos_enc:
            assert pos32 is not None and self.rope_narrow is not None
            zero_pos, rope_tab = pos32, self.rope_narrow
        x = self.ws("valf_x", (R, Cv))
        xpA, xpB = self.wsp("valf_xpA", R, Cv), self.wsp("valf_xpB", R, Cv)
        stA, stB = self.stats("valf_stA", R, Cv), self.stats("valf_stB", R, Cv)
        ops.copy2d(tok.reshape(R, Cv), Cv, x, Cv, R, Cv)
        ops.pack_stats(x, xpA, stA, rows=R, C_=Cv)
        for i in range(cfg.val_depth):
            self._block(x, xpA, stA, xpB, stB, R, B, P, Cv, cfg.enc_heads, "val%d." % i, zero_pos, tag="_valf",
                        head_dim=Cv // cfg.enc_heads, rope_tab=rope_tab)
        ops.gemm(xpA, w["value_out.w"], out, M=R, N=E, K=Cv, lda=Cv, ldc=E, bias=w["value_out.b"], res1=res, ldr1=E,
                 ln=ops.LnFold(stA, Cv, w["value_out.s"], 1e-6))
        return out

    def encode_cur_value(self, pts3d, out, res):
        self.activate()
        cfg, w = self.cfg, self.w
        B, H, W_, _ = pts3d.shape
        p, E = cfg.patch, cfg.enc_dim
        nh, nw = H // p, W_ // p
        P = nh * nw
        R = B * P
        _, pos32, zero_pos = self.positions(B, nh, nw)
        col = self.wsp("im2col_val", R, 3 * p * p)
        sb, sy, sx, sc = pts3d.stride()
        ops.im2col_patch(pts3d, col, B=B, C_=3, H=H, W_=W_, p=p, strides=(sb, sc, sy, sx))
        x, xp, st = self._vit(col, R, B, P, "pospatch", "val", cfg.val_depth, pos32 if cfg.mem_pos_enc else zero_pos, tag="_val")
        ops.gemm(xp, w["value_out.w"], out, M=R, N=E, K=E, lda=E, ldc=E, bias=w["value_out.b"], res1=res, ldr1=E,
                 ln=ops.LnFold(st, E, w["value_out.s"], 1e-6))
        return out
```

spann3r_amd/lib.py:

```python
import ctypes as C
import os

import torch

_HERE = os.path.dirname(os.path.abspath(__file__))
LIB_PATH = os.environ.get("SP3_LIB_PATH") or os.path.join(_HERE, "libspann3r_hip.so")

F32, BF16 = 0, 1
ACT_NONE, ACT_GELU, ACT_RELU = 0, 1, 2
EPI_PLAIN, EPI_ROPE_VT, EPI_PIXSHUF, EPI_PARTIAL = 0, 1, 2, 3
LOAD_PLAIN, LOAD_CONV3X3, LOAD_SOFTMAX = 0, 1, 2


class GemmDesc(C.Structure):
    _fields_ = [
        ("A", C.c_void_p), ("A2", C.c_void_p), ("W", C.c_void_p), ("C", C.c_void_p), ("bias", C.c_void_p),
        ("res1", C.c_void_p), ("res2", C.c_void_p),
        ("M", C.c_int32), ("N", C.c_int32), ("K", C.c_int32), ("batch", C.c_int32),
        ("K1", C.c_int32),
        ("lda", C.c_int64), ("lda2", C.c_int64), ("ldw", C.c_int64), ("ldc", C.c_int64),
        ("ldr1", C.c_int64), ("ldr2", C.c_int64),
        ("strideA", C.c_int64), ("strideW", C.c_int64), ("strideC", C.c_int64),
        ("alpha", C.c_float), ("wdtype", C.c_int32), ("act", C.c_int32), ("out_bf16", C.c_int32),
        ("relu_in", C.c_int32), ("loader", C.c_int32),
        ("conv_H", C.c_int32), ("conv_W", C.c_int32), ("conv_C", C.c_int32),
        ("conv_OH", C.c_int32), ("conv_OW", C.c_int32), ("conv_stride", C.c_int32),
        ("epi", C.c_int32),
        ("rope_cos", C.c_void_p), ("rope_sin", C.c_void_p), ("pos", C.c_void_p),
        ("rope_cols", C.c_int32), ("vt", C.c_void_p), ("tokens", C.c_int32), ("heads", C.c_int32),
        ("vt_ld", C.c_int64),
        ("ps_k", C.c_int32), ("ps_H", C.c_int32), ("ps_W", C.c_int32), ("ps_C", C.c_int32),
        ("tile", C.c_int32), ("a_bf16", C.c_int32), ("splitk", C.c_int32), ("a_packed", C.c_int32),
        ("ln_stats", C.c_void_p), ("ln_s", C.c_void_p), ("ln_nt", C.c_int32), ("ln_C", C.c_int32), ("ln_eps", C.c_float),
        ("stats_out", C.c_void_p), ("c2", C.c_void_p), ("qkv_packed", C.c_int32), ("out_packed", C.c_int32), ("w_packed", C.c_int32),
        ("sb_A2", C.c_int64), ("sb_bias", C.c_int64), ("sb_ln_stats", C.c_int64), ("sb_ln_s", C.c_int64),
        ("sb_stats_out", C.c_int64), ("sb_c2", C.c_int64), ("sb_vt", C.c_int64),
        ("trace", C.c_void_p),
        ("sm_stats_out", C.c_void_p), ("sm_stats", C.c_void_p), ("sm_nt", C.c_int32), ("sm_thresh", C.c_float), ("sm_zout", C.c_void_p),
        ("f32x3", C.c_int32), ("res_bf16", C.c_int32), ("dyn_n", C.c_void_p),
    ]


class HeadPart(C.Structure):
    _fields_ = [
        ("src", C.c_void_p), ("s_b", C.c_int64), ("s_n", C.c_int64), ("s_h", C.c_int64),
        ("dst", C.c_void_p), ("d_b", C.c_int64), ("d_n", C.c_int64), ("d_h", C.c_int64),
        ("dstT", C.c_void_p), ("pos", C.c_void_p), ("N", C.c_int32), ("fwd", C.c_float), ("ldT", C.c_int64),
    ]


class AttnBwdDesc(C.Structure):
    _fields_ = ([(n, C.c_void_p) for n in ("q", "k", "v", "dout")]
                + [(n, C.c_int64) for n in ("sq", "ldq", "sk", "ldk", "sv", "ldv", "sdo", "lddo")]
                + [(n, C.c_void_p) for n in ("qT", "kT", "doT")] + [("ldTq", C.c_int64), ("ldTk", C.c_int64)]
                + [("lse", C.c_void_p), ("D", C.c_void_p), ("dq", C.c_void_p), ("dk", C.c_void_p), ("dv", C.c_void_p)]
                + [(n, C.c_int64) for n in ("sdq", "lddq", "sdk", "lddk", "sdv", "lddv")]
                + [("B", C.c_int32), ("heads", C.c_int32), ("Nq", C.c_int32), ("Nk", C.c_int32), ("scale", C.c_float), ("bf16_products", C.c_int32)])


class AttnQProjDesc(C.Structure):
    _fields_ = [
        ("x_packed", C.c_void_p), ("x_group_stride", C.c_int64), ("ln_stats", C.c_void_p), ("stats_group_stride", C.c_int64),
        ("w_packed", C.c_void_p), ("w_group_stride", C.c_int64), ("ln_s", C.c_void_p), ("bias", C.c_void_p), ("vec_group_stride", C.c_int64),
        ("pos", C.c_void_p), ("rope_cos", C.c_void_p), ("rope_sin", C.c_void_p), ("ln_eps", C.c_float), ("D", C.c_int32),
        ("kp", C.c_void_p), ("k_cols", C.c_int32), ("k_col0", C.c_int32), ("npad_k", C.c_int32), ("vtp", C.c_void_p),
        ("out", C.c_void_p), ("ldo", C.c_int64), ("out_bf16", C.c_int32), ("out_packed", C.c_int32),
        ("B", C.c_int32), ("heads", C.c_int32), ("Nq", C.c_int32), ("Nk", C.c_int32), ("scale", C.c_float),
        ("o_group", C.c_int32), ("o_group_rows", C.c_int32),
    ]


class ReduceLnDesc(C.Structure):
    _fields_ = [
        ("partial", C.c_void_p), ("split_stride", C.c_int64), ("bias", C.c_void_p), ("res", C.c_void_p),
        ("ldres", C.c_int64), ("x_out", C.c_void_p), ("ldx", C.c_int64),
        ("g1", C.c_void_p), ("b1", C.c_void_p), ("out1", C.c_void_p), ("ld1", C.c_int64), ("out1_bf16", C.c_int32),
        ("g2", C.c_void_p), ("b2", C.c_void_p), ("out2", C.c_void_p), ("ld2", C.c_int64), ("out2_bf16", C.c_int32),
        ("eps", C.c_float), ("splits", C.c_int32), ("rows", C.c_int32), ("C", C.c_int32),
        ("out1_packed", C.c_int32), ("out2_packed", C.c_int32),
            ("act", C.c_int32), ("res2", C.c_void_p), ("ldres2", C.c_int64),
    ]


class BankWriteDesc(C.Structure):
    _fields_ = [
        ("feat_k", C.c_void_p), ("feat_v", C.c_void_p), ("k_raw", C.c_void_p), ("v_raw", C.c_void_p),
        ("k_hat", C.c_void_p), ("v_hat_t", C.c_void_p), ("s_bank", C.c_void_p), ("b_bank", C.c_void_p),
        ("gamma_k", C.c_void_p), ("beta_k", C.c_void_p), ("gamma_v", C.c_void_p), ("beta_v", C.c_void_p),
        ("gamma_q", C.c_void_p), ("beta_q", C.c_void_p),
        ("eps", C.c_float), ("alpha", C.c_float),
        ("M", C.c_int32), ("P", C.c_int32), ("C", C.c_int32), ("cap", C.c_int32), ("wdtype", C.c_int32), ("state", C.c_void_p),
    ]


_lib = None

_PROTOS = {
    "sp3_gemm": [C.POINTER(GemmDesc), C.c_void_p],
    "sp3_gemm2": [C.POINTER(GemmDesc), C.POINTER(GemmDesc), C.c_void_p],
    "sp3_gemm_plan": [C.POINTER(GemmDesc)],
    "sp3_layernorm": [C.c_void_p, C.c_int64, C.c_void_p, C.c_void_p, C.c_float, C.c_void_p, C.c_int64, C.c_int,
                      C.c_int, C.c_int, C.c_void_p],
    "sp3_reduce_ln": [C.POINTER(ReduceLnDesc), C.c_void_p],
    "sp3_layernorm_dual": [C.c_void_p, C.c_int64, C.c_void_p, C.c_void_p, C.c_float, C.c_void_p, C.c_int64, C.c_void_p, C.c_int, C.c_int,
                           C.c_int, C.c_int, C.c_void_p],
    "sp3_layernorm_packed": [C.c_void_p, C.c_int64, C.c_void_p, C.c_void_p, C.c_float, C.c_void_p, C.c_int,
                             C.c_int, C.c_int, C.c_void_p],
    "sp3_attention_ex": [C.c_void_p, C.c_int64, C.c_int64, C.c_void_p, C.c_int64, C.c_int64, C.c_void_p, C.c_int64,
                         C.c_void_p, C.c_int64, C.c_int, C.c_int, C.c_int, C.c_int, C.c_int, C.c_int, C.c_float, C.c_int,
                         C.c_void_p],
    "sp3_layernorm_t": [C.c_void_p, C.c_int64, C.c_void_p, C.c_void_p, C.c_float, C.c_void_p, C.c_int64, C.c_int,
                        C.c_int, C.c_int, C.c_void_p],
    "sp3_rope_2d": [C.c_void_p, C.c_int, C.c_int, C.c_int, C.c_int, C.c_int, C.c_int64, C.c_int64, C.c_int64,
                    C.c_void_p, C.c_float, C.c_float, C.c_void_p],
    "sp3_attention": [C.c_void_p, C.c_int64, C.c_int64, C.c_void_p, C.c_int64, C.c_int64, C.c_void_p, C.c_int64,
                      C.c_void_p, C.c_int64, C.c_int, C.c_int, C.c_int, C.c_int, C.c_int, C.c_float, C.c_int, C.c_void_p],
    "sp3_attention_packed": [C.c_void_p, C.c_int, C.c_int, C.c_int, C.c_void_p, C.c_int, C.c_int, C.c_int, C.c_void_p,
                             C.c_void_p, C.c_int64, C.c_int, C.c_int, C.c_int, C.c_int, C.c_int, C.c_int, C.c_float, C.c_int, C.c_int,
                             C.c_void_p],
    "sp3_attention_packed_qproj": [C.POINTER(AttnQProjDesc), C.c_void_p],
    "sp3_softmax_thresh": [C.c_void_p, C.c_void_p, C.c_int64, C.c_int64, C.c_int, C.c_int, C.c_int, C.c_float,
                           C.c_int, C.c_void_p, C.c_int64, C.c_int, C.c_void_p],
    "sp3_softmax_pack": [C.c_void_p, C.c_int64, C.c_int64, C.c_int, C.c_int, C.c_float, C.c_int, C.c_void_p, C.c_int64, C.c_int, C.c_void_p,
                         C.c_void_p],
    "sp3_colsum_packed": [C.c_void_p, C.c_int, C.c_int, C.c_int, C.c_void_p, C.c_void_p],
    "sp3_colsum_softmax": [C.c_void_p, C.c_int64, C.c_int, C.c_int, C.c_void_p, C.c_float, C.c_void_p, C.c_void_p, C.c_int, C.c_void_p],
    "sp3_bank_write": [C.POINTER(BankWriteDesc), C.c_void_p],
    "sp3_pack_stats": [C.c_void_p, C.c_int64, C.c_int, C.c_int, C.c_void_p, C.c_int, C.c_void_p, C.c_void_p],
    "sp3_gather_packed_rows": [C.c_void_p, C.c_void_p, C.c_void_p, C.c_int, C.c_int, C.c_int, C.c_void_p],
    "sp3_gather_packed_cols": [C.c_void_p, C.c_void_p, C.c_void_p, C.c_int, C.c_int, C.c_int, C.c_int, C.c_int, C.c_void_p],
    "sp3_colsum_accum": [C.c_void_p, C.c_int64, C.c_int, C.c_int, C.c_void_p, C.c_void_p],
    "sp3_cos_sim": [C.c_void_p, C.c_void_p, C.c_int, C.c_int, C.c_int, C.c_void_p, C.c_void_p, C.c_void_p],
    "sp3_mem_append": [C.c_void_p, C.c_void_p, C.c_int, C.c_int, C.c_void_p],
    "sp3_bank_state_set": [C.c_void_p, C.c_int, C.c_int, C.c_void_p],
    "sp3_prob_merge": [C.c_void_p, C.c_void_p, C.c_int, C.c_int, C.c_int, C.c_void_p, C.c_void_p],
    "sp3_colsum_prob": [C.c_void_p, C.c_void_p, C.c_int, C.c_int, C.c_int, C.c_void_p, C.c_void_p, C.c_void_p],
    "sp3_cos_sim_state": [C.c_void_p, C.c_void_p, C.c_int, C.c_int, C.c_int, C.c_void_p, C.c_void_p, C.c_void_p, C.c_void_p],
    "sp3_prune_select": [C.c_void_p, C.c_void_p, C.c_int, C.c_float, C.c_int, C.c_void_p, C.c_void_p],
    "sp3_gather_rows": [C.c_void_p, C.c_void_p, C.c_void_p, C.c_int, C.c_int, C.c_int, C.c_void_p],
    "sp3_gather_cols": [C.c_void_p, C.c_int64, C.c_void_p, C.c_int64, C.c_void_p, C.c_int, C.c_int, C.c_int,
                        C.c_int, C.c_void_p],
    "sp3_gather_1d": [C.c_void_p, C.c_void_p, C.c_void_p, C.c_int, C.c_void_p],
    "sp3_im2col_patch": [C.c_void_p, C.c_int64, C.c_int64, C.c_int64, C.c_int64, C.c_int, C.c_int, C.c_int, C.c_int,
                         C.c_int, C.c_void_p, C.c_int, C.c_int, C.c_void_p],
    "sp3_conv3x3_tile": [C.c_void_p, C.c_int, C.c_void_p, C.c_void_p, C.c_void_p, C.c_void_p, C.c_void_p, C.c_int, C.c_int, C.c_int,
                         C.c_int, C.c_int, C.c_int, C.c_int, C.c_int, C.c_void_p],
    "sp3_upsample2x": [C.c_void_p, C.c_void_p, C.c_int, C.c_int, C.c_int, C.c_int, C.c_int, C.c_int, C.c_void_p],
    "sp3_head_final": [C.c_void_p, C.c_void_p, C.c_void_p, C.c_int64, C.c_int, C.c_void_p, C.c_void_p, C.c_void_p,
                       C.c_void_p],
    "sp3_upsample2x_bf16": [C.c_void_p, C.c_void_p, C.c_int, C.c_int, C.c_int, C.c_int, C.c_int, C.c_int, C.c_void_p],
    "sp3_head_final_bf16": [C.c_void_p, C.c_void_p, C.c_void_p, C.c_int64, C.c_int, C.c_void_p, C.c_void_p, C.c_void_p,
                            C.c_void_p],
    "sp3_fill_f32": [C.c_void_p, C.c_float, C.c_int64, C.c_void_p],
    "sp3_cast_f32_to_bf16": [C.c_void_p, C.c_void_p, C.c_int64, C.c_void_p],
    "sp3_copy2d_f32": [C.c_void_p, C.c_int64, C.c_void_p, C.c_int64, C.c_int, C.c_int, C.c_void_p],
    "sp3_spin": [C.c_int64, C.c_void_p, C.c_void_p],
    "sp3_conf_loss_forward": [C.c_void_p, C.c_void_p, C.c_void_p, C.c_void_p, C.c_void_p, C.c_int, C.c_int, C.c_int, C.c_float, C.c_int,
                              C.c_void_p, C.c_void_p, C.c_void_p, C.c_void_p],
    "sp3_conf_loss_backward": [C.c_void_p, C.c_void_p, C.c_void_p, C.c_void_p, C.c_void_p, C.c_int, C.c_int, C.c_int, C.c_float, C.c_int,
                               C.c_void_p, C.c_void_p, C.c_void_p, C.c_void_p, C.c_void_p],
    "sp3_transpose": [C.c_void_p, C.c_int64, C.c_void_p, C.c_int64, C.c_int, C.c_int, C.c_void_p],
    "sp3_transpose_batched": [C.c_void_p, C.c_int64, C.c_int64, C.c_void_p, C.c_int64, C.c_int64, C.c_int, C.c_int, C.c_int, C.c_void_p],
    "sp3_transpose_pad": [C.c_void_p, C.c_int64, C.c_int64, C.c_void_p, C.c_int64, C.c_int64, C.c_int, C.c_int, C.c_int, C.c_int, C.c_void_p],
    "sp3_softmax_bwd_pad": [C.c_void_p, C.c_void_p, C.c_void_p, C.c_void_p, C.c_int64, C.c_int, C.c_int, C.c_int, C.c_float, C.c_void_p],
    "sp3_head_shuffle": [C.c_void_p, C.c_int, C.c_int, C.c_int, C.c_int, C.c_float, C.c_void_p, C.c_void_p, C.c_int, C.c_void_p],
    "sp3_attention_train_fwd": [C.c_void_p, C.c_int64, C.c_int64, C.c_void_p, C.c_int64, C.c_int64, C.c_void_p, C.c_int64, C.c_void_p, C.c_int64,
                                C.c_void_p, C.c_int, C.c_int, C.c_int, C.c_int, C.c_float, C.c_int, C.c_void_p],
    "sp3_attention_train_bwd": [C.c_void_p, C.c_void_p],
    "sp3_gelu": [C.c_void_p, C.c_void_p, C.c_int64, C.c_void_p],
    "sp3_gelu_bwd": [C.c_void_p, C.c_void_p, C.c_void_p, C.c_int64, C.c_void_p],
    "sp3_im2col3x3": [C.c_void_p, C.c_void_p, C.c_int, C.c_int, C.c_int, C.c_int, C.c_int, C.c_void_p],
    "sp3_col2im3x3": [C.c_void_p, C.c_void_p, C.c_int, C.c_int, C.c_int, C.c_int, C.c_int, C.c_void_p],
    "sp3_relu": [C.c_void_p, C.c_void_p, C.c_int64, C.c_void_p],
    "sp3_relu_bwd": [C.c_void_p, C.c_void_p, C.c_void_p, C.c_int64, C.c_void_p],
    "sp3_upsample2x_bwd": [C.c_void_p, C.c_void_p, C.c_int, C.c_int, C.c_int, C.c_int, C.c_int, C.c_int, C.c_void_p],
    "sp3_postprocess": [C.c_void_p, C.c_void_p, C.c_void_p, C.c_int64, C.c_void_p],
    "sp3_postprocess_bwd": [C.c_void_p, C.c_void_p, C.c_void_p, C.c_void_p, C.c_int64, C.c_void_p],
    "sp3_adamw": [C.c_void_p, C.c_void_p, C.c_void_p, C.c_void_p, C.c_int64, C.c_float, C.c_float, C.c_float, C.c_float, C.c_float, C.c_int,
                  C.c_float, C.c_void_p],
    "sp3_mul": [C.c_void_p, C.c_void_p, C.c_void_p, C.c_int64, C.c_void_p],
    "sp3_pack_bf16": [C.c_void_p, C.c_int64, C.c_int, C.c_int, C.c_void_p, C.c_void_p, C.c_void_p],
    "sp3_pack_bf16_conv3x3": [C.c_void_p, C.c_int, C.c_int, C.c_int, C.c_int, C.c_int, C.c_int, C.c_void_p, C.c_void_p, C.c_void_p],
# ... 72 lines not shown
```

spann3r_amd/ops.py:

```python
import ctypes as C

import torch

from . import lib as L
from .lib import GemmDesc, F32, BF16, ACT_NONE, ACT_GELU, ACT_RELU


_prof = None


class Profiler:

    def __init__(self, blocker_ms=12.0):
        self.rec = []
        self.regions = []
        self.blocker_cycles = int(blocker_ms * 2.4e6)

    def step_begin(self):
        torch.cuda._sleep(self.blocker_cycles)

    def region_begin(self):
        return (self.begin(), len(self.rec))

    def region_end(self, key, e0, nbytes, info=None):
# ... 27 lines not shown
        self.step_begin()
        ev = []
        for i in range(n):
            e0 = torch.cuda.Event(enable_timing=True)
            e1 = torch.cuda.Event(enable_timing=True)
            e0.record()
            L.check(L.load().sp3_spin(12000, ticks[i:].data_ptr(), L.stream_ptr()), "sp3_spin")
            e1.record()
            ev.append((e0, e1))
        torch.cuda.synchronize()
        dur_ms = (ticks.cpu().double() * 1e-5).tolist()
        t = sorted(a.elapsed_time(b) - d for (a, b), d in zip(ev, dur_ms))
        self.bracket_ms = max(t[len(t) // 2], 0.0)
        return self.bracket_ms

    def summary(self):
        torch.cuda.synchronize()
        agg = {}
        ov = getattr(self, "bracket_ms", 0.0)
        for key, e0, e1, fl, by in self.rec:
            a = agg.setdefault(key, dict(launches=0, ms=0.0, flops=0.0, bytes=0.0))
            a["launches"] += 1
            a["ms"] += max(e0.elapsed_time(e1) - ov, 1e-4)
            a["flops"] += fl
            a["bytes"] += by
        return agg


def set_profiler(p):
    global _prof
    _prof = p


_TILE_NAMES = {0: "32x32xk4", 1: "64x64", 2: "64x128", 3: "64x64xk4", 4: "32x64xk4", 18: "16x64xk4", 5: "128x128lds", 6: "128x64lds", 7: "112x64lds",
               8: "208x64lds", 9: "112x32lds", 10: "112x64lds2w", 11: "112x64lds8w", 12: "208x64lds8w", 13: "112x64wreg8",
               14: "112x64wreg4", 15: "208x64wreg8", 16: "112x64wreg4l6", 17: "112x64wreg8l4",
               20: "256x128pipe", 21: "128x128pipe", 22: "128x64pipe", 23: "64x64pipe", 24: "64x32pipe", 25: "32x32pipe",
               30: "lean-rope-k1024-48x64xk8", 31: "lean-rope-k768-32x32xk4", 32: "lean-packed-k1024-64x64xk8", 33: "lean-packed-k768-32x32xk4",
               34: "lean-stream-k1024-32x32xk8", 35: "lean-stream-k4096-32x32xk8r4", 36: "lean-stream-k768-48x32xk6",
               37: "lean-stream-k3072-48x32xk8", 38: "lean-stream-k1792-64x32xk7",
               39: "lean-stream-k1024-48x32xk8", 40: "lean-conv-16x16xk12", 41: "lean-conv-32x32xk8", 42: "lean-packed-splitA-k1792-64x32xk7", 43: "lean-score-k1024-32x32xk8", 44: "lean-softmax-pv-16x64xk8",
               45: "lean-prob-k1024-256x128", 46: "lean-prob-pv-256x128",
               50: "lean-rope-k1024-256x128", 51: "lean-rope-k1024-128x128", 52: "lean-rope-k768-128x128", 53: "lean-packed-k1024-256x128",
               54: "lean-packed-k1024-128x128", 55: "lean-packed-k768-128x128", 56: "lean-stream-k1024-128x64", 57: "lean-stream-k4096-128x64",
               58: "lean-stream-k768-128x64", 59: "lean-stream-k3072-128x64", 60: "lean-stream-k1792-128x64",
               61: "lean-stream-k1024-256x128", 62: "lean-stream-k4096-256x128", 63: "lean-rope-k768-256x128", 64: "lean-packed-k768-256x128", 65: "lean-rope-k768-128x64", 66: "lean-packed-splitA-k1792-128x128", 67: "lean-packed-splitA-k1792-256x128"}


def pick_tile(M, N, batch=1, splitk=1, conv=False, K=0, packed_bf16=False, plain=False, ln_nt=0, pipe_ok=False, rope=False):
    t64 = ((M + 63) // 64) * ((N + 63) // 64) * batch * splitk
    t128 = ((M + 63) // 64) * ((N + 127) // 128) * batch
    lds_ok = not conv and splitk == 1 and packed_bf16 and K % 64 == 0
    wide_legacy = lds_ok and M >= 1024 and N >= 2304 and N % 128 == 0 and N < 16384
    if pipe_ok and PIPE_TILES and M >= 512 and not rope and not wide_legacy:
        mt256, mt128, nt128 = (M + 255) // 256, (M + 127) // 128, (N + 127) // 128
        if mt256 * nt128 * batch * splitk >= 144:
            return 20
        if mt128 * nt128 * batch * splitk >= 200:
            return 21
        if mt128 * ((N + 63) // 64) * batch * splitk <= 192:
            return 24
        return 22
    if lds_ok and M >= 1024 and N >= 2304 and N % 128 == 0:
        return 5 if (N % 4096 == 0 or ((M + 127) // 128) * (N // 128) * batch >= 1024) else 6
    if not conv and M >= 1024:
        return 1
    if lds_ok and 112 < M <= 224 and plain and N >= 3072 and K <= 1024 and ln_nt <= 32:
        return 13
    if conv or M > 2048:
        if t128 >= 1024 and N % 128 == 0:
            return 2
        if t64 >= 512:
            return 1
        return 0
    return 0


import os as _os
import threading as _threading
PIPE_TILES = True
PROF_SHAPES = _os.environ.get("SP3_PROF_SHAPES", "0")[:1] == "1"
LEAN = _os.environ.get("SP3_LEAN_GEMM", "1")[:1] != "0"

_pair = None


class pair:

    def __enter__(self):
        global _pair
        assert _pair is None
        _pair = []
        return self

    def __exit__(self, et, ev, tb):
        global _pair
        descs, _pair = _pair, None
        if et is not None:
            return False
        if len(descs) != 2:
            raise RuntimeError("ops.pair(): expected exactly two GEMM launches, got %d" % len(descs))
        (a, na), (b, _) = descs
        if a.tile < 0 and b.tile < 0:
            ta, tb = L.load().sp3_gemm_plan(C.byref(a)), L.load().sp3_gemm_plan(C.byref(b))
            if ta >= 30 and ta == tb and a.epi == L.EPI_ROPE_VT and b.epi == L.EPI_ROPE_VT:
                a.tile = b.tile = ta
        if a.tile < 0:
            _pick_general(a)
        if b.tile < 0:
            b.tile = a.tile
        if _prof is None:
            L.check(L.load().sp3_gemm2(C.byref(a), C.byref(b), L.stream_ptr()), "sp3_gemm2")
            return False
        e0 = _prof.begin()
        L.check(L.load().sp3_gemm2(C.byref(a), C.byref(b), L.stream_ptr()), "sp3_gemm2")
        fl, by = 0.0, 0.0
        for d in (a, b):
            f, n = _gemm_cost(d)
            fl, by = fl + f, by + n
        _prof.end("gemm2<A%s,W%s,%s,%s>" % ("bf16" if a.a_bf16 else "f32", "f32" if a.wdtype == F32 else "bf16", na, _TILE_NAMES[a.tile]), e0, fl, by)
        return False


def _pipe_ok(d):
    return bool(d.loader == L.LOAD_PLAIN and d.a_packed and d.w_packed and d.a_bf16 and not d.A2 and not d.sm_stats_out and d.K % 64 == 0
                and (max(d.splitk, 1) == 1 or d.epi == L.EPI_PARTIAL))


def _pick_general(d):
    d.tile = pick_tile(d.M, d.N, max(d.batch, 1), max(d.splitk, 1), d.loader == L.LOAD_CONV3X3, d.K,
                       bool(d.a_packed and d.w_packed and d.a_bf16 and not d.A2 and d.epi != L.EPI_PARTIAL
                            and not d.sm_stats_out),
                       d.epi == L.EPI_PLAIN, d.ln_nt if d.ln_stats else 0, _pipe_ok(d), d.epi == L.EPI_ROPE_VT)


def _pick(d):
    t = L.load().sp3_gemm_plan(C.byref(d))
    if t >= 30:
        d.tile = t
        return
    _pick_general(d)


def _gemm_cost(d):
    b = max(d.batch, 1)
    wsz = 4 if d.wdtype == F32 else 2
    asz, csz = (2 if d.a_bf16 else 4), (2 if d.out_bf16 else 4)
    a_elems = d.M * d.K if d.loader != L.LOAD_CONV3X3 else d.M * d.conv_stride * d.conv_stride * d.conv_C
    return 2.0 * d.M * d.N * d.K * b, b * (asz * a_elems + wsz * d.N * d.K + csz * d.M * d.N)


def _gemm_launch(d, what, loader_name):
    if _pair is not None:
        _pair.append((d, loader_name))
        return
    if d.loader == L.LOAD_SOFTMAX:
        if d.tile < 0:
            t = L.load().sp3_gemm_plan(C.byref(d))
            d.tile = t if t >= 30 else 0
        elif d.tile < 30:
            d.tile = 1 if d.tile == 1 else 0
    if d.tile < 0:
        _pick(d)
    if _prof is None:
        L.check(L.load().sp3_gemm(C.byref(d), L.stream_ptr()), what)
        return
    e0 = _prof.begin()
# ... 162 lines not shown
    d.batch, d.strideA, d.strideW, d.strideC = batch, strideA, strideW, strideC
    for k, v in (sb or {}).items():
        setattr(d, "sb_" + k, v)


def wdtype_of(t):
    if t.dtype == torch.float32:
        return F32
    if t.dtype == torch.bfloat16:
        return BF16
    raise TypeError("weights must be float32 or bfloat16, got %s" % t.dtype)


def _f32(t, name):
    if t is not None and (t.dtype != torch.float32 or not t.is_cuda):
        raise TypeError("%s must be a float32 CUDA(HIP) tensor" % name)


def _is_packed(t):
    return int(isinstance(t, PackedAct))


def _act(t, name):
    if not t.is_cuda or t.dtype not in (torch.float32, torch.bfloat16):
        raise TypeError("%s must be a float32/bfloat16 CUDA(HIP) tensor" % name)
    return int(t.dtype == torch.bfloat16)


def gemm(A, W, out, *, M, N, K, lda, ldc, bias=None, res1=None, ldr1=0, res2=None, ldr2=0, act=ACT_NONE, alpha=1.0,
         relu_in=False, tile=-1, batch=1, strideA=0, strideW=0, strideC=0, ldw=0,
         A2=None, lda2=0, K1=0, splitk=0, ln=None, stats_out=None, c2=None, sb=None, trace=None,
         sm_stats_out=None, softmax=None, plan_only=False, dyn_n=None):
    d = GemmDesc()
    d.a_bf16 = _act(A, "A")
    d.a_packed = _is_packed(A)
    d.out_packed = _is_packed(out)
    out_bf16 = out.dtype == torch.bfloat16
    _w(d, W)
    d.A, d.A2, d.C = A.data_ptr(), L.ptr(A2), out.data_ptr()
    d.bias, d.res1, d.res2 = L.ptr(bias), L.ptr(res1), L.ptr(res2)
    d.M, d.N, d.K, d.batch, d.K1 = M, N, K, batch, K1
    d.lda, d.lda2, d.ldw, d.ldc, d.ldr1, d.ldr2 = lda, lda2, ldw, ldc, ldr1, ldr2
    d.strideA, d.strideW, d.strideC = strideA, strideW, strideC
    d.alpha, d.act, d.out_bf16, d.relu_in = alpha, act, int(out_bf16), int(relu_in)
    d.loader, d.epi, d.tile = L.LOAD_PLAIN, L.EPI_PLAIN, tile
    if splitk >= 1:
        d.epi, d.splitk = L.EPI_PARTIAL, splitk
    _ln(d, ln)
    d.stats_out, d.c2 = L.ptr(stats_out), L.ptr(c2)
    d.trace = L.ptr(trace)
    d.sm_stats_out = L.ptr(sm_stats_out)
    d.dyn_n = L.ptr(dyn_n)
    if softmax is not None:
        st, thresh, zout = softmax
        d.loader, d.sm_stats, d.sm_nt, d.sm_thresh, d.sm_zout = L.LOAD_SOFTMAX, st.data_ptr(), (K + 31) // 32, float(thresh), L.ptr(zout)
    if sb:
        _group(d, batch, strideA, strideW, strideC, sb)
    if plan_only:
        return int(L.load().sp3_gemm_plan(C.byref(d)))
    _gemm_launch(d, "sp3_gemm", "softmax" if softmax is not None else "plain")
    return out


def reduce_ln(partial, splits, rows, C_, *, bias=None, res=None, ldres=0, x_out=None, ldx=0,
              ln1=None, out1=None, ld1=0, ln2=None, out2=None, ld2=0, eps=1e-6, act=ACT_NONE, res2=None, ldres2=0):
    d = L.ReduceLnDesc()
    d.partial, d.split_stride, d.splits, d.rows, d.C = partial.data_ptr(), rows * C_, splits, rows, C_
    d.bias, d.res, d.ldres = L.ptr(bias), L.ptr(res), ldres or C_
    d.x_out, d.ldx = L.ptr(x_out), ldx or C_
    d.act, d.res2, d.ldres2 = act, L.ptr(res2), ldres2 or C_
    if out1 is not None:
        d.g1, d.b1, d.out1, d.ld1, d.out1_bf16 = ln1[0].data_ptr(), ln1[1].data_ptr(), out1.data_ptr(), ld1 or C_, int(out1.dtype == torch.bfloat16)
        d.out1_packed = _is_packed(out1)
    if out2 is not None:
        d.g2, d.b2, d.out2, d.ld2, d.out2_bf16 = ln2[0].data_ptr(), ln2[1].data_ptr(), out2.data_ptr(), ld2 or C_, int(out2.dtype == torch.bfloat16)
        d.out2_packed = _is_packed(out2)
    d.eps = eps
    nln = (out1 is not None) + (out2 is not None)
    _timed("reduce_ln", (splits + 8.0 * nln) * rows * C_, 4.0 * rows * C_ * (splits + 2 + nln),
           lambda: L.check(L.load().sp3_reduce_ln(C.byref(d), L.stream_ptr()), "sp3_reduce_ln"))


def conv3x3(x, Wp, out, *, B, H, W_, Cin, Cout, stride=1, bias=None, res1=None, res2=None, act=ACT_NONE,
            relu_in=False, tile=-1, force_tile_kernel=False, splitk_ws=None, tile_px=None):
    OH, OW = (H - 1) // stride + 1, (W_ - 1) // stride + 1
    if (tile < 0 and stride == 1 and isinstance(Wp, PackedWeight) and Wp.dtype == torch.bfloat16
            and Cin % 64 == 0 and Cout % 64 == 0 and Cin <= 768 and (force_tile_kernel or B * H * W_ >= 2048)):
        _act(x, "x")
        rbf = [t.dtype == torch.bfloat16 for t in (res1, res2) if t is not None]
        if rbf and (any(rbf) != all(rbf) or (any(rbf) and out.dtype != torch.bfloat16)):
            raise TypeError("conv3x3: residual maps must share one dtype (bf16 only next to a bf16 output)")
        oflag = int(out.dtype == torch.bfloat16) | (2 if any(rbf) else 0) | ({None: 0, "8x8": 1, "8x16": 2, "8x16n32": 3}[tile_px] << 2)
        _timed("conv3x3_tile", 2.0 * B * H * W_ * Cout * 9 * Cin,
               B * H * W_ * (x.element_size() * Cin + out.element_size() * Cout) + 2.0 * 9 * Cin * Cout,
               lambda: L.check(L.load().sp3_conv3x3_tile(
                   x.data_ptr(), int(x.dtype == torch.bfloat16), Wp.data_ptr(), L.ptr(bias), L.ptr(res1), L.ptr(res2),
                   out.data_ptr(), oflag, B, H, W_, Cin, Cout, int(relu_in), act,
                   L.stream_ptr()), "sp3_conv3x3_tile"))
        return out
    d = GemmDesc()
    d.a_bf16 = _act(x, "x")
    d.out_bf16 = int(out.dtype == torch.bfloat16)
    _w(d, Wp)
    M = B * OH * OW
    lean = -1
    if tile < 0 and isinstance(Wp, PackedWeight):
        p = GemmDesc()
        p.a_bf16, p.out_bf16 = d.a_bf16, d.out_bf16
        _w(p, Wp)
        p.A, p.C, p.bias, p.res1, p.res2 = x.data_ptr(), out.data_ptr(), L.ptr(bias), L.ptr(res1), L.ptr(res2)
        p.M, p.N, p.K, p.batch = M, Cout, 9 * Cin, 1
        p.lda, p.ldc, p.ldr1, p.ldr2 = Cin, Cout, Cout, Cout
        p.alpha, p.act, p.relu_in = 1.0, act, int(relu_in)
        p.loader, p.epi, p.tile = L.LOAD_CONV3X3, L.EPI_PLAIN, -1
        p.conv_H, p.conv_W, p.conv_C, p.conv_OH, p.conv_OW, p.conv_stride = H, W_, Cin, OH, OW, stride
        rbf = [t.dtype == torch.bfloat16 for t in (res1, res2) if t is not None]
        if rbf and any(rbf) != all(rbf):
            raise TypeError("conv3x3: residual maps must share one dtype")
        p.res_bf16 = int(any(rbf))
        lean = L.load().sp3_gemm_plan(C.byref(p))
        if lean >= 30:
            p.tile = lean
            _gemm_launch(p, "sp3_gemm(conv3x3)", "conv3x3")
            return out
    if any(t is not None and t.dtype == torch.bfloat16 for t in (res1, res2)):
        raise TypeError("conv3x3: bf16 residual maps are served by the lean small-map and the LDS-tiled kernels only "
                        "(B*H*W=%d, Cin=%d, Cout=%d, stride %d)" % (B * H * W_, Cin, Cout, stride))
    S = conv_splitk(M, Cout, 9 * Cin, Wp.dtype) if (splitk_ws is not None and tile < 0 and out.dtype == torch.float32) else 1
    if S > 1 and splitk_ws.numel() < S * M * Cout:
        raise ValueError("conv3x3: splitk_ws holds %d floats, needs %d" % (splitk_ws.numel(), S * M * Cout))
    d.A, d.C = x.data_ptr(), (splitk_ws if S > 1 else out).data_ptr()
    if S == 1:
        d.bias, d.res1, d.res2 = L.ptr(bias), L.ptr(res1), L.ptr(res2)
    d.M, d.N, d.K, d.batch = M, Cout, 9 * Cin, 1
    d.lda, d.ldc, d.ldr1, d.ldr2 = Cin, Cout, Cout, Cout
    d.alpha, d.act, d.relu_in = 1.0, (act if S == 1 else ACT_NONE), int(relu_in)
    d.loader, d.epi, d.tile = L.LOAD_CONV3X3, (L.EPI_PLAIN if S == 1 else L.EPI_PARTIAL), (tile if S == 1 else 0)
    d.splitk = S if S > 1 else 0
    d.conv_H, d.conv_W, d.conv_C, d.conv_OH, d.conv_OW, d.conv_stride = H, W_, Cin, OH, OW, stride
    _gemm_launch(d, "sp3_gemm(conv3x3)", "conv3x3")
    if S > 1:
        reduce_ln(splitk_ws, S, M, Cout, bias=bias, res=res1, ldres=Cout, x_out=out, ldx=Cout, act=act, res2=res2, ldres2=Cout)
    return out


def conv_splitk(M, N, K, wdtype):
    tiles = ((M + 31) // 32) * ((N + 31) // 32)
    nkb = K // (64 if wdtype == torch.bfloat16 else 32)
    s = 1
    while tiles * s * 2 <= 512 and nkb // (s * 2) >= 4 and s < 8:
        s *= 2
    return s


def conv_transpose_ks(x, Wp, out, *, B, H, W_, Cin, Cout, ks, bias=None, tile=-1):
    d = GemmDesc()
    d.a_bf16 = _act(x, "x")
    d.out_bf16 = int(out.dtype == torch.bfloat16)
    _w(d, Wp)
    d.A, d.C, d.bias = x.data_ptr(), out.data_ptr(), L.ptr(bias)
    d.M, d.N, d.K, d.batch = B * H * W_, ks * ks * Cout, Cin, 1
    d.lda, d.ldc = Cin, Cout
    d.alpha = 1.0
    d.loader, d.epi, d.tile = L.LOAD_PLAIN, L.EPI_PIXSHUF, tile
    d.ps_k, d.ps_H, d.ps_W, d.ps_C = ks, H, W_, Cout
    _gemm_launch(d, "sp3_gemm(conv_transpose)", "plain")
    return out


def proj_rope_vt(A, W, bias, out_qk, ldc, vt, vt_ld, *, M, N, K, lda, rope_cols, pos, cos, sin, tokens, heads, tile=-1,
                 qkv_packed=False, ln=None, batch=1, strideA=0, strideW=0, strideC=0, sb=None):
    d = GemmDesc()
    d.a_bf16 = _act(A, "A")
    d.a_packed = _is_packed(A)
    _w(d, W)
    d.A, d.C, d.bias = A.data_ptr(), L.ptr(out_qk), L.ptr(bias)
    d.M, d.N, d.K, d.batch = M, N, K, 1
    d.lda, d.ldc = lda, ldc
    d.alpha = 1.0
    d.loader, d.epi, d.tile = L.LOAD_PLAIN, L.EPI_ROPE_VT, tile
    d.rope_cos, d.rope_sin, d.pos, d.rope_cols = cos.data_ptr(), sin.data_ptr(), pos.data_ptr(), rope_cols
    d.vt, d.vt_ld, d.tokens, d.heads = L.ptr(vt), vt_ld, tokens, heads
    d.qkv_packed = int(qkv_packed)
    _ln(d, ln)
    if out_qk is None:
        d.C = vt.data_ptr()
    if batch > 1:
        _group(d, batch, strideA, strideW, strideC, sb)
    _gemm_launch(d, "sp3_gemm(rope_vt)", "plain")


def layernorm(x, gamma, beta, eps, out, *, rows, C_, ldx=None, ldo=None, transposed=False, dual=None, group_rows=0):
    _f32(x, "x")
    ldx = C_ if ldx is None else ldx
    ldo = C_ if ldo is None else ldo
    if dual is not None:
        assert dual.dtype == torch.bfloat16 and not transposed and not _is_packed(out)
        pad = getattr(dual, "rows_pad", (group_rows + 15) // 16 * 16)
        _timed("layernorm", 8.0 * rows * C_, rows * C_ * 10.0,
               lambda: L.check(L.load().sp3_layernorm_dual(x.data_ptr(), ldx, gamma.data_ptr(), beta.data_ptr(), eps, out.data_ptr(), ldo,
                                                           dual.data_ptr(), rows, C_, group_rows or rows, pad, L.stream_ptr()),
                               "sp3_layernorm_dual"))
        return out
    if _is_packed(out):
        _timed("layernorm", 8.0 * rows * C_, rows * C_ * 6.0,
               lambda: L.check(L.load().sp3_layernorm_packed(x.data_ptr(), ldx, gamma.data_ptr(), beta.data_ptr(), eps,
                                                             out.data_ptr(), int(out.dtype == torch.bfloat16), rows, C_,
                                                             L.stream_ptr()), "sp3_layernorm_packed"))
        return out
    fn = L.load().sp3_layernorm_t if transposed else L.load().sp3_layernorm
    _timed("layernorm_t" if transposed else "layernorm", 8.0 * rows * C_, rows * C_ * (4.0 + out.element_size()),
           lambda: L.check(fn(x.data_ptr(), ldx, gamma.data_ptr(), beta.data_ptr(), eps, out.data_ptr(), ldo,
                              int(out.dtype == torch.bfloat16), rows, C_, L.stream_ptr()), "sp3_layernorm"))
    return out


def rope_2d(tokens, positions, base, fwd):
    if tokens.dim() != 4:
        raise RuntimeError("tokens must have 4 dimensions")
    if positions.dim() != 3:
        raise RuntimeError("positions must have 3 dimensions")
    if tokens.size(0) != positions.size(0):
        raise RuntimeError("batch size differs between tokens & positions")
    if tokens.size(1) != positions.size(1):
        raise RuntimeError("seq_length differs between tokens & positions")
    if positions.size(2) != 2:
# ... 260 lines not shown
```

Before: 628.9.

## Batch DPT head small-map convs into level launches and fuse 2x upsample into residual

Generalizes the paired GEMM launch to up to four descriptors and adds a conv-level kernel that runs several independent small-map 3x3 convolutions of a DPT head level in one launch, ordered by cost. It also lets the lean conv epilogue read a half-resolution res2 and bilinearly upsample it on the fly, replacing a separate upsample pass and its intermediate map. The intent is fewer kernel launches and less HBM traffic in the head, at the cost of a larger kernel argument struct, more per-block group selection, and new ordering constraints in the Python head.

Result: faster. 639.9, median of 6 (+1.7%).

```diff
diff --git a/include/spann3r_hip.h b/include/spann3r_hip.h
--- a/include/spann3r_hip.h
+++ b/include/spann3r_hip.h
@@ -69,9 +69,11 @@
   int32_t f32x3;
   int32_t res_bf16;
   const int32_t* dyn_n;
+  int32_t res2_up_H, res2_up_W;
 } sp3_gemm_desc;
 int sp3_gemm(const sp3_gemm_desc* desc_host, void* stream);
 int sp3_gemm2(const sp3_gemm_desc* a, const sp3_gemm_desc* b, void* stream);
+int sp3_gemm_n(const sp3_gemm_desc* const* descs, int n, void* stream);
 int sp3_gemm_plan(const sp3_gemm_desc* desc_host);
 
 int sp3_layernorm(const float* x, int64_t ldx, const float* gamma, const float* beta, float eps,
diff --git a/spann3r_amd/csrc/common.h b/spann3r_amd/csrc/common.h
--- a/spann3r_amd/csrc/common.h
+++ b/spann3r_amd/csrc/common.h
@@ -83,6 +83,29 @@
 template <typename T> __device__ __forceinline__ void st_out(T* p, T v) { *p = v; }
 #endif
 
+struct Up2xTaps {
+  int p00, p01, p10, p11;
+  float hy, ly, hx, lx;
+};
+__device__ __forceinline__ Up2xTaps up2x_taps(int H, int W, int oy, int ox) {
+  const int OH = 2 * H, OW = 2 * W;
+  const float sh = OH > 1 ? (float)(H - 1) / (float)(OH - 1) : 0.f;
+  const float sw = OW > 1 ? (float)(W - 1) / (float)(OW - 1) : 0.f;
+  int y0 = (int)__fmul_rn(sh, (float)oy), x0 = (int)__fmul_rn(sw, (float)ox);
+  y0 = y0 < H - 1 ? y0 : H - 1;
+  x0 = x0 < W - 1 ? x0 : W - 1;
+  const int y1 = y0 < H - 1 ? y0 + 1 : y0, x1 = x0 < W - 1 ? x0 + 1 : x0;
+  Up2xTaps t;
+  t.ly = __fmaf_rn(sh, (float)oy, -(float)y0); t.lx = __fmaf_rn(sw, (float)ox, -(float)x0);
+  t.hy = 1.f - t.ly; t.hx = 1.f - t.lx;
+  t.p00 = y0 * W + x0; t.p01 = y0 * W + x1; t.p10 = y1 * W + x0; t.p11 = y1 * W + x1;
+  return t;
+}
+__device__ __forceinline__ float up2x_mix(const Up2xTaps& t, float v00, float v01, float v10, float v11) {
+  const float top = __fmaf_rn(t.hx, v00, __fmul_rn(t.lx, v01)), bot = __fmaf_rn(t.hx, v10, __fmul_rn(t.lx, v11));
+  return __fmaf_rn(t.hy, top, __fmul_rn(t.ly, bot));
+}
+
 __device__ __forceinline__ int64_t packed_off(int row, int k, int K, bool bf16) {
   const int lkb = bf16 ? 6 : 5, lch = bf16 ? 4 : 3;
   const int nkb = (K + (1 << lkb) - 1) >> lkb;
diff --git a/spann3r_amd/csrc/gemm.hip b/spann3r_amd/csrc/gemm.hip
--- a/spann3r_amd/csrc/gemm.hip
+++ b/spann3r_amd/csrc/gemm.hip
@@ -6,9 +6,8 @@
 namespace {
 
 struct GemmArgs {
-  sp3_gemm_desc d;
-  sp3_gemm_desc d2;
-  int nb1;
+  sp3_gemm_desc dn[4];
+  int nb[4];
   int xcd_slices;
 };
 
@@ -395,8 +394,10 @@
 template <typename TA, typename TW, int LOADER, int MF, int NF, int WM, int WN, int WK, int STAGES, int LOOP = 0, int XM = 0>
 __global__ __launch_bounds__(64 * (WM * WN * WK + (LOOP >= 2 ? LOOP : 0)), (gemm_min_waves<TA, LOADER, MF, NF, WK>()))
 void gemm_kernel(const GemmArgs args) {
-  const bool second = args.nb1 > 0 && (int)blockIdx.y >= args.nb1;
-  sp3_gemm_desc d = second ? args.d2 : args.d;
+  int grp = 0;
+#pragma unroll
+  for (int i = 1; i < 4; ++i) grp = (int)blockIdx.y >= args.nb[i] ? i : grp;
+  sp3_gemm_desc d = args.dn[grp];
   using M_ = MM<TA, TW>;
   constexpr bool LDSK = LOOP != 0;
   constexpr int NCW = WM * WN * WK;
@@ -428,7 +429,7 @@
   const int tid = threadIdx.x, lane = tid & 63, wave = tid >> 6;
   const int wk = wave % WK, wn = (wave / WK) % WN, wm = wave / (WK * WN);
   const int g = lane >> 4;
-  const int bz = second ? (int)blockIdx.y - args.nb1 : (int)blockIdx.y;
+  const int bz = (int)blockIdx.y - args.nb[grp];
   if (d.batch > 1) {
     auto shift = [&](auto*& p, int64_t bytes) {
       using P = std::remove_reference_t<decltype(p)>;
@@ -444,7 +445,7 @@
   const TW* W = reinterpret_cast<const TW*>(d.W) + (int64_t)bz * d.strideW;
 
   const int m0 = tile_m * BM, n0 = tile_n * BN;
-  int64_t* tr0 = ((LOOP == 0 || LOOP == -1) && args.d.trace && blockIdx.x < 8 && blockIdx.y == 0 && blockIdx.z == 0 && threadIdx.x == 0) ? args.d.trace + blockIdx.x * 64 : nullptr;
+  int64_t* tr0 = ((LOOP == 0 || LOOP == -1) && d.trace && blockIdx.x < 8 && blockIdx.y == 0 && blockIdx.z == 0 && threadIdx.x == 0) ? d.trace + blockIdx.x * 64 : nullptr;
   if (tr0) { tr0[0] = clock64(); tr0[3] = wall_clock64(); }
   ARows<TA, LOADER, MF> arows;
   arows.init(d, A, m0 + wm * MF * 16, lane, M_::KB, M_::CH);
@@ -1464,7 +1465,8 @@
   if (tr0) { tr0[2] = clock64(); tr0[4] = wall_clock64(); }
 }
 
-thread_local const sp3_gemm_desc* g_pair = nullptr;
+thread_local const sp3_gemm_desc* g_more[3] = {nullptr, nullptr, nullptr};
+thread_local int g_nmore = 0;
 
 template <typename TA, typename TW, int LOADER, int MF, int NF, int WM, int WN, int WK, int STAGES, int LOOP = 0, int XM = 0>
 int launch(const sp3_gemm_desc& d, hipStream_t stream) {
@@ -1490,17 +1492,20 @@
     }
   }
   GemmArgs a;
-  a.d = d;
-  a.nb1 = 0;
+  a.dn[0] = d;
+  a.nb[0] = 0;
   int gy = d.batch;
-  if (g_pair) {
-    a.d2 = *g_pair;
-    a.nb1 = d.batch;
-    gy += g_pair->batch;
-    const int b2 = grid_x(*g_pair);
-    blocks = blocks > b2 ? blocks : b2;
-  } else {
-    a.d2 = d;
+  for (int i = 1; i < 4; ++i) {
+    if (i <= g_nmore) {
+      a.dn[i] = *g_more[i - 1];
+      a.nb[i] = gy;
+      gy += g_more[i - 1]->batch;
+      const int b2 = grid_x(*g_more[i - 1]);
+      blocks = blocks > b2 ? blocks : b2;
+    } else {
+      a.dn[i] = d;
+      a.nb[i] = 0x7fffffff;
+    }
   }
   a.xcd_slices = (gy == 1 && d.splitk >= 8 && d.splitk % 8 == 0 && blocks % 8 == 0) ? 1 : 0;
   hipLaunchKernelGGL(kern, dim3(blocks, gy, d.splitk), dim3(NT), lds, stream, a);
@@ -1734,6 +1739,7 @@
   if (d.tile >= 30 || (d.tile < 0 && sp3_gemm_sm_tile(d) >= 0)) return sp3_gemm_sm_launch(d, nullptr, reinterpret_cast<hipStream_t>(stream_));
   SP3_CHECK(!(d.a_packed && d.A2), "sp3_gemm: a fragment-order A split along K runs on the lean instances only (no instance for M=%d N=%d K=%d)", d.M, d.N, d.K);
   SP3_CHECK(!(d.res_bf16 && (d.res1 || d.res2)), "sp3_gemm: bf16 residual maps are read by the lean small-map convolutions only (res_bf16 = out_bf16 = a_bf16; M=%d N=%d K=%d)", d.M, d.N, d.K);
+  SP3_CHECK(!d.res2_up_H, "sp3_gemm: a half-resolution res2 is read by the lean small-map convolutions only (tiles 40 / 41; M=%d N=%d K=%d)", d.M, d.N, d.K);
   SP3_CHECK(!d.dyn_n, "sp3_gemm: a device-side extent (dyn_n) is served by the lean memory-read instances only (tiles 43 / 44; M=%d N=%d K=%d)", d.M, d.N, d.K);
   return gemm_dispatch(d, tile, reinterpret_cast<hipStream_t>(stream_));
 }
@@ -1748,30 +1754,52 @@
   return lean >= 0 ? lean : tile;
 }
 
+extern "C" int sp3_gemm_n(const sp3_gemm_desc* const* dp, int n, void* stream_) {
+  SP3_CHECK(dp != nullptr && n >= 1 && n <= 4, "sp3_gemm_n: 1..4 descriptors (n=%d)", n);
+  for (int i = 0; i < n; ++i) SP3_CHECK(dp[i] != nullptr, "sp3_gemm_n: null descriptor");
+  if (n == 1) return sp3_gemm(dp[0], stream_);
+  hipStream_t stream = reinterpret_cast<hipStream_t>(stream_);
+  sp3_gemm_desc d[4];
+  int t[4] = {-1, -1, -1, -1};
+  {
+    sp3_gemm_desc d0[4];
+    const int want = dp[0]->tile;
+    bool ok = true;
+    for (int i = 0; i < n; ++i) {
+      d0[i] = *dp[i];
+      const int keep = d0[i].tile;
+      d0[i].tile = -1;
+      int ti = -1;
+      ok = ok && gemm_prepare(d0[i], ti) == 0;
+      if (d0[i].loader == SP3_LOAD_CONV3X3) d0[i].tile = keep;
+    }
+    if (ok && sp3_gemm_sm_conv_level(d0, n)) return sp3_gemm_sm_conv_level_launch(d0, n, stream);
+    if (ok && n == 2) {
+      d0[0].tile = d0[1].tile = -1;
+      const int la = sp3_gemm_sm_tile(d0[0]), lb = sp3_gemm_sm_tile(d0[1]);
+      if (la >= 30 && la == lb && sp3_gemm_sm_pairs(d0[0]) && (want < 0 || want == la)) return sp3_gemm_sm_launch(d0[0], &d0[1], stream);
+    }
+    SP3_CHECK(want < 30, "sp3_gemm_n: tile %d asks for a lean instance that does not take these %d groups", want, n);
+  }
+  for (int i = 0; i < n; ++i) {
+    d[i] = *dp[i];
+    if (i > 0 && d[i].tile < 0) d[i].tile = t[0];
+    if (int rc = gemm_prepare(d[i], t[i])) return rc;
+    SP3_CHECK(!(d[i].res_bf16 && (d[i].res1 || d[i].res2)) && !d[i].res2_up_H, "sp3_gemm_n: bf16 and half-resolution residual maps are read by the lean small-map convolutions only");
+    SP3_CHECK(t[i] == t[0] && d[i].wdtype == d[0].wdtype && d[i].a_bf16 == d[0].a_bf16 && d[i].loader == d[0].loader && d[i].loader != SP3_LOAD_SOFTMAX &&
+              d[i].f32x3 == d[0].f32x3 && (d[i].w_packed == 2) == (d[0].w_packed == 2),
+              "sp3_gemm_n: every group must use one kernel instance (tile %d / %d, same dtypes and loader)", t[0], t[i]);
+    SP3_CHECK(d[i].splitk == 1 && !d[i].trace && !d[i].dyn_n, "sp3_gemm_n: no split-K, no trace, no device-side extent");
+  }
+  for (int i = 1; i < n; ++i) g_more[i - 1] = &d[i];
+  g_nmore = n - 1;
+  const int rc = gemm_dispatch(d[0], t[0], stream);
+  g_nmore = 0;
+  return rc;
+}
+
 extern "C" int sp3_gemm2(const sp3_gemm_desc* ap, const sp3_gemm_desc* bp, void* stream_) {
   SP3_CHECK(ap != nullptr && bp != nullptr, "sp3_gemm2: null descriptor");
-  sp3_gemm_desc a = *ap, b = *bp;
-  int ta = -1, tb = -1;
-  {
-    sp3_gemm_desc a0 = a, b0 = b;
-    int t0 = -1, t1 = -1;
-    const int want = a0.tile;
-    a0.tile = b0.tile = -1;
-    if (gemm_prepare(a0, t0) == 0 && gemm_prepare(b0, t1) == 0) {
-      const int la = sp3_gemm_sm_tile(a0), lb = sp3_gemm_sm_tile(b0);
-      if (la >= 30 && la == lb && sp3_gemm_sm_pairs(a0) && (want < 0 || want == la)) return sp3_gemm_sm_launch(a0, &b0, reinterpret_cast<hipStream_t>(stream_));
-    }
-    SP3_CHECK(want < 30, "sp3_gemm2: tile %d asks for a lean instance that does not take this pair", want);
-  }
-  if (int rc = gemm_prepare(a, ta)) return rc;
-  if (b.tile < 0) b.tile = ta;
-  if (int rc = gemm_prepare(b, tb)) return rc;
-  SP3_CHECK(!(a.res_bf16 && (a.res1 || a.res2)) && !(b.res_bf16 && (b.res1 || b.res2)), "sp3_gemm2: bf16 residual maps are read by the lean small-map convolutions only");
-  SP3_CHECK(ta == tb && a.wdtype == b.wdtype && a.a_bf16 == b.a_bf16 && a.loader == b.loader && a.loader != SP3_LOAD_SOFTMAX,
-            "sp3_gemm2: both groups must use one kernel instance (tile %d / %d, same dtypes and loader)", ta, tb);
-  SP3_CHECK(a.splitk == 1 && b.splitk == 1 && !a.trace && !b.trace && !a.dyn_n && !b.dyn_n, "sp3_gemm2: no split-K, no trace, no device-side extent");
-  g_pair = &b;
-  const int rc = gemm_dispatch(a, ta, reinterpret_cast<hipStream_t>(stream_));
-  g_pair = nullptr;
-  return rc;
+  const sp3_gemm_desc* two[2] = {ap, bp};
+  return sp3_gemm_n(two, 2, stream_);
 }
diff --git a/spann3r_amd/csrc/gemm_sm.h b/spann3r_amd/csrc/gemm_sm.h
--- a/spann3r_amd/csrc/gemm_sm.h
+++ b/spann3r_amd/csrc/gemm_sm.h
@@ -4,3 +4,5 @@
 int sp3_gemm_sm_tile(const sp3_gemm_desc& d);
 bool sp3_gemm_sm_pairs(const sp3_gemm_desc& d);
 int sp3_gemm_sm_launch(const sp3_gemm_desc& d, const sp3_gemm_desc* pair, hipStream_t stream);
+bool sp3_gemm_sm_conv_level(const sp3_gemm_desc* ds, int n);
+int sp3_gemm_sm_conv_level_launch(const sp3_gemm_desc* ds, int n, hipStream_t stream);
diff --git a/spann3r_amd/csrc/gemm_sm.hip b/spann3r_amd/csrc/gemm_sm.hip
--- a/spann3r_amd/csrc/gemm_sm.hip
+++ b/spann3r_amd/csrc/gemm_sm.hip
@@ -1146,6 +1146,13 @@
   const float* bias; const void* res1; const void* res2;
   int M, N, H, Wd, Cin, OH, OW, stride, nkb, relu_in, act;
   unsigned cin_magic, per_magic, ow_magic;
+  int up_H, up_W;
+};
+
+struct ConvLevelArgs {
+  ConvSmArgs p[4];
+  int start[5];
+  int tile[4];
 };
 
 typedef __attribute__((ext_vector_type(4))) unsigned int csm_u32x4;
@@ -1194,6 +1201,7 @@
   const bf16x4 t = *reinterpret_cast<const bf16x4*>(p);
   return make_float4((float)t[0], (float)t[1], (float)t[2], (float)t[3]);
 }
+template <typename TM> __device__ __forceinline__ float csm_round(float v) { return (float)(TM)v; }
 __device__ __forceinline__ void csm_store4(float* p, const float (&v)[4]) { st_out(reinterpret_cast<float4*>(p), make_float4(v[0], v[1], v[2], v[3])); }
 __device__ __forceinline__ void csm_store4(__bf16* p, const float (&v)[4]) {
   bf16x4 t;
@@ -1202,13 +1210,11 @@
 }
 
 template <typename TM, int MF, int NF, int WK, int R>
-__global__ __launch_bounds__(64 * WK) void conv_sm_kernel(const ConvSmArgs a) {
+__device__ __forceinline__ void conv_sm_body(const ConvSmArgs& a, const int tile_m, const int tile_n, float* smem) {
   constexpr int BM = MF * 16, BN = NF * 16, NT = 64 * WK, LD = BN + 4, CG = BN / 4;
-  extern __shared__ __attribute__((aligned(16))) float smem[];
   const int tid = threadIdx.x, lane = tid & 63, wk = __builtin_amdgcn_readfirstlane(tid >> 6);
-  const int tile_m = blockIdx.y, tile_n = blockIdx.z * 8 + blockIdx.x;
   const int m0 = tile_m * BM, n0 = tile_n * BN;
-  if (n0 >= a.N) return;
+  if (n0 >= a.N || wk >= WK) return;
   const int g = lane >> 4, r16 = lane & 15;
   const TM* X = reinterpret_cast<const TM*>(a.x);
 
@@ -1219,7 +1225,7 @@
     const long o = (long)(m0 + erow) * a.N + n0 + ec4;
     if (a.bias) b4 = *reinterpret_cast<const float4*>(a.bias + n0 + ec4);
     if (a.res1) r1 = csm_load4(reinterpret_cast<const TM*>(a.res1) + o);
-    if (a.res2) r2 = csm_load4(reinterpret_cast<const TM*>(a.res2) + o);
+    if (a.res2 && !a.up_H) r2 = csm_load4(reinterpret_cast<const TM*>(a.res2) + o);
   }
 
   const TM* img[MF];
@@ -1312,8 +1318,43 @@
 #pragma unroll
       for (int e = 0; e < 4; ++e) v[e] = fmaxf(v[e], 0.f);
     }
+    if (a.up_H) {
+      const int row = m0 + erow;
+      const int b = (int)__umulhi((unsigned)row, a.per_magic), rem = row - b * a.OH * a.OW;
+      const int oy = (int)__umulhi((unsigned)rem, a.ow_magic), ox = rem - oy * a.OW;
+      const Up2xTaps up = up2x_taps(a.up_H, a.up_W, oy, ox);
+      const TM* src = reinterpret_cast<const TM*>(a.res2) + (long)b * a.up_H * a.up_W * a.N + n0 + ec4;
+      const float4 u00 = csm_load4(src + (long)up.p00 * a.N), u01 = csm_load4(src + (long)up.p01 * a.N);
+      const float4 u10 = csm_load4(src + (long)up.p10 * a.N), u11 = csm_load4(src + (long)up.p11 * a.N);
+      r2.x = csm_round<TM>(up2x_mix(up, u00.x, u01.x, u10.x, u11.x)); r2.y = csm_round<TM>(up2x_mix(up, u00.y, u01.y, u10.y, u11.y));
+      r2.z = csm_round<TM>(up2x_mix(up, u00.z, u01.z, u10.z, u11.z)); r2.w = csm_round<TM>(up2x_mix(up, u00.w, u01.w, u10.w, u11.w));
+    }
     v[0] += r1.x + r2.x; v[1] += r1.y + r2.y; v[2] += r1.z + r2.z; v[3] += r1.w + r2.w;
     csm_store4(reinterpret_cast<TM*>(a.out) + (long)(m0 + erow) * a.N + n0 + ec4, v);
+  }
+}
+
+template <typename TM, int MF, int NF, int WK, int R>
+__global__ __launch_bounds__(64 * WK) void conv_sm_kernel(const ConvSmArgs a) {
+  extern __shared__ __attribute__((aligned(16))) float smem[];
+  conv_sm_body<TM, MF, NF, WK, R>(a, blockIdx.y, blockIdx.z * 8 + blockIdx.x, smem);
+}
+
+template <typename TM>
+__global__ __launch_bounds__(64 * 12) void conv_level_kernel(const ConvLevelArgs a) {
+  extern __shared__ __attribute__((aligned(16))) float smem[];
+  const int w = blockIdx.x;
+  int p = 0;
+#pragma unroll
+  for (int i = 1; i < 4; ++i) p = w >= a.start[i] ? i : p;
+  const ConvSmArgs q = a.p[p];
+  const int local = w - a.start[p], j = local >> 3;
+  if (a.tile[p] == 40) {
+    const int mt = (q.M + 15) / 16;
+    conv_sm_body<TM, 1, 1, 12, 3>(q, j % mt, (j / mt) * 8 + (local & 7), smem);
+  } else if constexpr (sizeof(TM) == 2) {
+    const int mt = (q.M + 31) / 32;
+    conv_sm_body<TM, 2, 2, 8, 3>(q, j % mt, (j / mt) * 8 + (local & 7), smem);
   }
 }
 
@@ -1336,11 +1377,13 @@
   if (d.ldc != d.N || (d.res1 && d.ldr1 != d.N) || (d.res2 && d.ldr2 != d.N) || (d.ldw > 0 && d.ldw != d.K)) return -1;
   if ((d.res1 || d.res2) && (d.res_bf16 != 0) != (d.out_bf16 != 0)) return -1;
   if (d.conv_OW < 2 || d.conv_OH * d.conv_OW < 2 || d.conv_C < 2) return -1;
+  if ((d.res2_up_H != 0) != (d.res2_up_W != 0) || d.res2_up_H < 0 || (d.res2_up_H && !d.out_bf16) ||
+      (d.res2 && d.res2_up_H && (d.conv_OH > 2 * d.res2_up_H || d.conv_OW > 2 * d.res2_up_W))) return -1;
   if (d.M <= 256) return d.N % 16 == 0 ? 40 : -1;
   return d.N % 32 == 0 ? 41 : -1;
 }
 
-int conv_sm_dispatch(const sp3_gemm_desc& d, int tile, hipStream_t stream) {
+ConvSmArgs conv_sm_args(const sp3_gemm_desc& d) {
   ConvSmArgs a;
   a.x = d.A; a.W = reinterpret_cast<const char*>(d.W); a.out = d.C;
   a.bias = d.bias; a.res1 = d.res1; a.res2 = d.res2;
@@ -1348,12 +1391,49 @@
   a.stride = d.conv_stride; a.nkb = d.K / 64; a.relu_in = d.relu_in; a.act = d.act;
   auto magic = [](int v) { return (unsigned)((1ull << 32) / (unsigned)v + 1); };
   a.cin_magic = magic(d.conv_C); a.per_magic = magic(d.conv_OH * d.conv_OW); a.ow_magic = magic(d.conv_OW);
+  a.up_H = d.res2 ? d.res2_up_H : 0; a.up_W = d.res2 ? d.res2_up_W : 0;
+  return a;
+}
+
+int conv_sm_dispatch(const sp3_gemm_desc& d, int tile, hipStream_t stream) {
+  const ConvSmArgs a = conv_sm_args(d);
   if (d.a_bf16) {
     if (tile == 40) return conv_sm_launch<__bf16, 1, 1, 12, 3>(a, stream);
     return conv_sm_launch<__bf16, 2, 2, 8, 3>(a, stream);
   }
   if (tile == 40) return conv_sm_launch<float, 1, 1, 12, 3>(a, stream);
   return conv_sm_launch<float, 2, 2, 8, 3>(a, stream);
+}
+
+int conv_level_dispatch(const sp3_gemm_desc* ds, int n, hipStream_t stream) {
+  ConvLevelArgs a = {};
+  int order[4], cost[4];
+  for (int i = 0; i < n; ++i) {
+    order[i] = i;
+    cost[i] = conv_sm_tile(ds[i]) == 40 ? ds[i].K / 64 * 2 : ds[i].K / 64 * 3;
+  }
+  for (int i = 1; i < n; ++i)
+    for (int j = i; j > 0 && cost[order[j]] > cost[order[j - 1]]; --j) { const int t = order[j]; order[j] = order[j - 1]; order[j - 1] = t; }
+  size_t lds = 0;
+  int threads = 0;
+  for (int i = 0; i < n; ++i) {
+    const sp3_gemm_desc& d = ds[order[i]];
+    const int tile = conv_sm_tile(d);
+    const int bm = tile == 40 ? 16 : 32, wk = tile == 40 ? 12 : 8;
+    a.p[i] = conv_sm_args(d);
+    a.tile[i] = tile;
+    a.start[i + 1] = a.start[i] + 8 * ((d.M + bm - 1) / bm) * ((d.N / bm + 7) / 8);
+    const size_t l = (size_t)wk * bm * (bm + 4) * sizeof(float);
+    lds = l > lds ? l : lds;
+    threads = 64 * wk > threads ? 64 * wk : threads;
+  }
+  for (int i = n; i < 4; ++i) { a.p[i] = a.p[0]; a.tile[i] = a.tile[0]; a.start[i + 1] = 0x7fffffff; }
+  const int blocks = a.start[n];
+  if (n < 4) a.start[n] = 0x7fffffff;
+  if (ds[0].a_bf16) hipLaunchKernelGGL(conv_level_kernel<__bf16>, dim3(blocks), dim3(threads), lds, stream, a);
+  else              hipLaunchKernelGGL(conv_level_kernel<float>, dim3(blocks), dim3(threads), lds, stream, a);
+  SP3_LAUNCH_CHECK("sp3_gemm_n (lean conv3x3 level)");
+  return 0;
 }
 
 struct SmInst {
@@ -1517,6 +1597,17 @@
   return s && s->epi == SM_ROPE;
 }
 
+bool sp3_gemm_sm_conv_level(const sp3_gemm_desc* ds, int n) {
+  if (!sm_enabled() || n < 2 || n > 4) return false;
+  for (int i = 0; i < n; ++i) {
+    const int t = conv_sm_tile(ds[i]);
+    if (t < 0 || (ds[i].tile >= 0 && ds[i].tile != t) || (ds[i].a_bf16 != 0) != (ds[0].a_bf16 != 0) || (t == 41 && !ds[i].a_bf16)) return false;
+  }
+  return true;
+}
+
+int sp3_gemm_sm_conv_level_launch(const sp3_gemm_desc* ds, int n, hipStream_t stream) { return conv_level_dispatch(ds, n, stream); }
+
 int sp3_gemm_sm_launch(const sp3_gemm_desc& d, const sp3_gemm_desc* pair, hipStream_t stream) {
   if (d.loader == SP3_LOAD_SOFTMAX && sm_enabled() && pvs_ok(d) && !pair && (d.tile < 30 || d.tile == 46)) return pvs_dispatch(d, stream);
   if (d.loader == SP3_LOAD_SOFTMAX) {
diff --git a/spann3r_amd/engine.py b/spann3r_amd/engine.py
--- a/spann3r_amd/engine.py
+++ b/spann3r_amd/engine.py
@@ -580,29 +580,37 @@
     def _conv_ws(self, head):
         return self.ws("conv_splitk_ws" + str(head), (1 << 23,))
 
-    def _rcu(self, x, pre, B, H, W_, out, extra_res=None, tag=""):
+    def _rcu_c1(self, x, pre, B, H, W_, tag=""):
         w, F = self.w, self.cfg.dpt_feat
         t = self.ws("rcu_tmp" + tag, (B * H * W_, F), self.mdt)
-        sk = self._conv_ws(tag[:1])
         ops.conv3x3(x, w[pre + "c1.w"], t, B=B, H=H, W_=W_, Cin=F, Cout=F, bias=w[pre + "c1.b"], relu_in=True, act=ACT_RELU,
-                    splitk_ws=sk)
+                    splitk_ws=self._conv_ws(tag[:1]))
+        return t
+
+    def _rcu(self, x, pre, B, H, W_, out, extra_res=None, tag="", c1_done=False, extra_up=None):
+        w, F = self.w, self.cfg.dpt_feat
+        t = self.ws("rcu_tmp" + tag, (B * H * W_, F), self.mdt)
+        if not c1_done:
+            self._rcu_c1(x, pre, B, H, W_, tag)
         ops.conv3x3(t, w[pre + "c2.w"], out, B=B, H=H, W_=W_, Cin=F, Cout=F, bias=w[pre + "c2.b"], res1=x, res2=extra_res,
-                    splitk_ws=sk)
+                    splitk_ws=self._conv_ws(tag[:1]), res2_up=extra_up)
         return out
 
-    def _fusion(self, pre, B, H, W_, x0, x1, tag, crop=None):
+    def _fusion(self, pre, B, H, W_, x0, x1, tag, crop=None, c1_done=False, x0_up=None, fold_up=False):
         w, F = self.w, self.cfg.dpt_feat
         M = B * H * W_
         cur = x0
         if x1 is not None:
             s = self.ws("fus_sum_" + tag, (M, F), self.mdt)
-            self._rcu(x1, pre + "u1", B, H, W_, s, extra_res=x0, tag=tag)
+            self._rcu(x1, pre + "u1", B, H, W_, s, extra_res=x0, tag=tag, c1_done=c1_done, extra_up=x0_up)
             cur = s
         r = self.ws("fus_rcu2_" + tag, (M, F), self.mdt)
-        self._rcu(cur, pre + "u2", B, H, W_, r, tag=tag)
+        self._rcu(cur, pre + "u2", B, H, W_, r, tag=tag, c1_done=c1_done and x1 is None)
         oc = self.ws("fus_oc_" + tag, (M, F), self.mdt)
         ops.gemm(r, w[pre + "out.w"], oc, M=M, N=F, K=F, lda=F, ldc=F, bias=w[pre + "out.b"])
         OH, OW = (2 * H, 2 * W_) if crop is None else crop
+        if fold_up:
+            return oc, OH, OW
         up = self.ws("fus_up_" + tag, (B * OH * OW, F), self.mdt)
         ops.upsample2x(oc, up, B=B, H=H, W_=W_, C_=F, outH=OH, outW=OW)
         return up, OH, OW
@@ -620,11 +628,14 @@
         t = [self.ws("dpt%d_pp%d" % (num, i), (R, ld[i]), mdt) for i in range(4)]
         pairable = len({dec[hk[i]].dtype for i in range(4)}) == 1
         import contextlib
+        lv = ops.HEAD_LEVELS
+        level = ops.level if lv else contextlib.nullcontext
         pair = ops.pair if pairable else contextlib.nullcontext
-        for i0 in (0, 2):
-            with pair():
-                for i in (i0, i0 + 1):
-                    ops.gemm(dec[hk[i]], w[pre + "pp%d.w" % i], t[i], M=R, N=ld[i], K=dims[i], lda=dims[i], ldc=ld[i], bias=w[pre + "pp%d.b" % i])
+        with (level if pairable else contextlib.nullcontext)():
+            for i0 in (0, 2):
+                with (contextlib.nullcontext if lv else pair)():
+                    for i in (i0, i0 + 1):
+                        ops.gemm(dec[hk[i]], w[pre + "pp%d.w" % i], t[i], M=R, N=ld[i], K=dims[i], lda=dims[i], ldc=ld[i], bias=w[pre + "pp%d.b" % i])
         c0 = 128 if self.wdt == torch.bfloat16 else ld[0]
         l0 = self.ws("dpt%d_l0" % num, (B * 16 * nh * nw, c0), mdt)
         l1 = self.ws("dpt%d_l1" % num, (B * 4 * nh * nw, ld[1]), mdt)
@@ -635,19 +646,42 @@
         h3, w3 = (nh - 1) // 2 + 1, (nw - 1) // 2 + 1
         l3 = self.ws("dpt%d_l3" % num, (B * h3 * w3, ld[3]), mdt)
         sk = self._conv_ws(num)
-        ops.conv3x3(t[3], w[pre + "pp3c.w"], l3, B=B, H=nh, W_=nw, Cin=ld[3], Cout=ld[3], stride=2, bias=w[pre + "pp3c.b"],
-                    splitk_ws=sk)
         geo = ((4 * nh, 4 * nw), (2 * nh, 2 * nw), (nh, nw), (h3, w3))
-        rn = []
-        for i, src in enumerate((l0, l1, l2, l3)):
-            Hh, Ww = geo[i]
-            o = self.ws("dpt%d_rn%d" % (num, i), (B * Hh * Ww, F), mdt)
-            ops.conv3x3(src, w[pre + "rn%d.w" % i], o, B=B, H=Hh, W_=Ww, Cin=(c0 if i == 0 else ld[i]), Cout=F, splitk_ws=sk)
-            rn.append(o)
-        p4, H4, W4 = self._fusion(pre + "ref4.", B, h3, w3, rn[3], None, "%d_4" % num, crop=(nh, nw))
-        p3, H3, W3 = self._fusion(pre + "ref3.", B, H4, W4, p4, rn[2], "%d_3" % num)
-        p2, H2, W2 = self._fusion(pre + "ref2.", B, H3, W3, p3, rn[1], "%d_2" % num)
-        p1, H1, W1 = self._fusion(pre + "ref1.", B, H2, W2, p2, rn[0], "%d_1" % num)
+        srcs = (l0, l1, l2, l3)
+        rn = [self.ws("dpt%d_rn%d" % (num, i), (B * geo[i][0] * geo[i][1], F), mdt) for i in range(4)]
+
+        def layer_rn(i):
+            ops.conv3x3(srcs[i], w[pre + "rn%d.w" % i], rn[i], B=B, H=geo[i][0], W_=geo[i][1], Cin=(c0 if i == 0 else ld[i]), Cout=F, splitk_ws=sk)
+
+        def pp3c():
+            ops.conv3x3(t[3], w[pre + "pp3c.w"], l3, B=B, H=nh, W_=nw, Cin=ld[3], Cout=ld[3], stride=2, bias=w[pre + "pp3c.b"], splitk_ws=sk)
+
+        refs = [(pre + "ref%d." % (4 - j), "%d_%d" % (num, 4 - j)) for j in range(4)]
+        if lv:
+            with level():
+                pp3c()
+                layer_rn(2)
+            with level():
+                layer_rn(0)
+                layer_rn(1)
+                layer_rn(3)
+                self._rcu_c1(rn[2], refs[1][0] + "u1", B, geo[2][0], geo[2][1], refs[1][1])
+            with level():
+                self._rcu_c1(rn[3], refs[0][0] + "u2", B, geo[3][0], geo[3][1], refs[0][1])
+                self._rcu_c1(rn[1], refs[2][0] + "u1", B, geo[1][0], geo[1][1], refs[2][1])
+                self._rcu_c1(rn[0], refs[3][0] + "u1", B, geo[0][0], geo[0][1], refs[3][1])
+        else:
+            pp3c()
+            for i in range(4):
+                layer_rn(i)
+        path, up, Hc, Wc = rn[3], None, h3, w3
+        for j in range(4):
+            Hn, Wn = geo[3 - j]
+            fold = lv and j < 3 and ops.conv3x3_takes_res2_up(w[refs[j + 1][0] + "u1c2.w"], mdt, B, *geo[2 - j])
+            nxt, OH_, OW_ = self._fusion(refs[j][0], B, Hn, Wn, path, rn[3 - j] if j else None, refs[j][1], crop=(nh, nw) if j == 0 else None,
+                                         c1_done=lv, x0_up=up, fold_up=fold)
+            path, up = nxt, ((Hn, Wn) if fold else None)
+        p1, H1, W1 = path, OH_, OW_
         a = self.ws("dpt%d_h0" % num, (B * H1 * W1, Lc), mdt)
         ops.conv3x3(p1, w[pre + "h0.w"], a, B=B, H=H1, W_=W1, Cin=F, Cout=Lc, bias=w[pre + "h0.b"])
         OH, OW = 2 * H1, 2 * W1
diff --git a/spann3r_amd/lib.py b/spann3r_amd/lib.py
--- a/spann3r_amd/lib.py
+++ b/spann3r_amd/lib.py
@@ -38,6 +38,7 @@
         ("trace", C.c_void_p),
         ("sm_stats_out", C.c_void_p), ("sm_stats", C.c_void_p), ("sm_nt", C.c_int32), ("sm_thresh", C.c_float), ("sm_zout", C.c_void_p),
         ("f32x3", C.c_int32), ("res_bf16", C.c_int32), ("dyn_n", C.c_void_p),
+        ("res2_up_H", C.c_int32), ("res2_up_W", C.c_int32),
     ]
 
 
@@ -98,6 +99,7 @@
 _PROTOS = {
     "sp3_gemm": [C.POINTER(GemmDesc), C.c_void_p],
     "sp3_gemm2": [C.POINTER(GemmDesc), C.POINTER(GemmDesc), C.c_void_p],
+    "sp3_gemm_n": [C.POINTER(C.POINTER(GemmDesc)), C.c_int, C.c_void_p],
     "sp3_gemm_plan": [C.POINTER(GemmDesc)],
     "sp3_layernorm": [C.c_void_p, C.c_int64, C.c_void_p, C.c_void_p, C.c_float, C.c_void_p, C.c_int64, C.c_int,
                       C.c_int, C.c_int, C.c_void_p],
diff --git a/spann3r_amd/ops.py b/spann3r_amd/ops.py
--- a/spann3r_amd/ops.py
+++ b/spann3r_amd/ops.py
@@ -133,7 +133,86 @@
 PROF_SHAPES = _os.environ.get("SP3_PROF_SHAPES", "0")[:1] == "1"
 LEAN = _os.environ.get("SP3_LEAN_GEMM", "1")[:1] != "0"
 
+HEAD_LEVELS = _os.environ.get("SP3_HEAD_LEVELS", "1")[:1] != "0"
 _pair = None
+
+
+def level_block_map(problems):
+    start = [0]
+    for tile, M, N in problems:
+        bm = 16 if tile == 40 else 32
+        start.append(start[-1] + 8 * ((M + bm - 1) // bm) * ((N // bm + 7) // 8))
+
+    def f(w):
+        p = max(i for i in range(len(problems)) if w >= start[i])
+        tile, M, N = problems[p]
+        bm = 16 if tile == 40 else 32
+        mt = (M + bm - 1) // bm
+        local = w - start[p]
+        j = local >> 3
+        return p, j % mt, (j // mt) * 8 + (local & 7)
+    return start[-1], f
+
+
+def level_order(problems):
+    cost = [(K // 64) * (2 if tile == 40 else 3) for tile, K in problems]
+    return sorted(range(len(problems)), key=lambda i: -cost[i])
+
+
+class level:
+
+    def __enter__(self):
+        global _pair
+        assert _pair is None
+        _pair = []
+        return self
+
+    def __exit__(self, et, ev, tb):
+        global _pair
+        descs, _pair = _pair, None
+        if et is not None:
+            return False
+        lean = [x for x in descs if x[0].loader == L.LOAD_CONV3X3]
+        conv = [x for x in lean if x[0].a_bf16 or x[0].tile == 40]
+        rest = [x for x in descs if x[0].loader != L.LOAD_CONV3X3]
+        if lean and rest:
+            raise RuntimeError("ops.level(): small-map convolutions and other GEMMs do not share a launch")
+        for x in lean:
+            if not any(x is y for y in conv):
+                self._send([x], True)
+        for group in (conv, rest):
+            for i in range(0, len(group), 4):
+                self._send(group[i:i + 4], group is conv)
+        return False
+
+    @staticmethod
+    def _send(group, is_conv):
+        if len(group) == 1:
+            _gemm_launch(group[0][0], "sp3_gemm", group[0][1])
+            return
+        ds = [g[0] for g in group]
+        if not is_conv:
+            for i in range(0, len(ds), 2):
+                if ds[i].tile < 0:
+                    _pick_general(ds[i])
+                for d in ds[i + 1:i + 2]:
+                    if d.tile < 0:
+                        d.tile = ds[i].tile
+            if len(ds) > 2 and len({d.tile for d in ds}) > 1:
+                for i in range(0, len(group), 2):
+                    level._send(group[i:i + 2], False)
+                return
+        arr = (C.POINTER(GemmDesc) * len(ds))(*[C.pointer(d) for d in ds])
+        e0 = _prof.begin() if _prof is not None else None
+        L.check(L.load().sp3_gemm_n(arr, len(ds), L.stream_ptr()), "sp3_gemm_n")
+        if _prof is not None:
+            fl, by = 0.0, 0.0
+            for d in ds:
+                f, n = _gemm_cost(d)
+                fl, by = fl + f, by + n
+            a = ds[0]
+            _prof.end("gemm_n<A%s,W%s,%s,%s x%d>" % ("bf16" if a.a_bf16 else "f32", "f32" if a.wdtype == F32 else "bf16", group[0][1],
+                                                     "+".join(sorted({_TILE_NAMES[d.tile] for d in ds})), len(ds)), e0, fl, by)
 
 
 class pair:
@@ -462,10 +541,12 @@
 
 
 def conv3x3(x, Wp, out, *, B, H, W_, Cin, Cout, stride=1, bias=None, res1=None, res2=None, act=ACT_NONE,
-            relu_in=False, tile=-1, force_tile_kernel=False, splitk_ws=None, tile_px=None):
+            relu_in=False, tile=-1, force_tile_kernel=False, splitk_ws=None, tile_px=None, res2_up=None):
     OH, OW = (H - 1) // stride + 1, (W_ - 1) // stride + 1
     if (tile < 0 and stride == 1 and isinstance(Wp, PackedWeight) and Wp.dtype == torch.bfloat16
             and Cin % 64 == 0 and Cout % 64 == 0 and Cin <= 768 and (force_tile_kernel or B * H * W_ >= 2048)):
+        if res2_up is not None:
+            raise ValueError("conv3x3: a half-resolution res2 is read by the lean small-map kernels only (B*H*W=%d)" % (B * H * W_))
         _act(x, "x")
         rbf = [t.dtype == torch.bfloat16 for t in (res1, res2) if t is not None]
         if rbf and (any(rbf) != all(rbf) or (any(rbf) and out.dtype != torch.bfloat16)):
@@ -498,11 +579,15 @@
         if rbf and any(rbf) != all(rbf):
             raise TypeError("conv3x3: residual maps must share one dtype")
         p.res_bf16 = int(any(rbf))
+        if res2_up is not None:
+            p.res2_up_H, p.res2_up_W = res2_up
         lean = L.load().sp3_gemm_plan(C.byref(p))
         if lean >= 30:
             p.tile = lean
             _gemm_launch(p, "sp3_gemm(conv3x3)", "conv3x3")
             return out
+    if res2_up is not None:
+        raise ValueError("conv3x3: a half-resolution res2 is read by the lean small-map kernels only (B*H*W=%d)" % (B * H * W_))
     if any(t is not None and t.dtype == torch.bfloat16 for t in (res1, res2)):
         raise TypeError("conv3x3: bf16 residual maps are served by the lean small-map and the LDS-tiled kernels only "
                         "(B*H*W=%d, Cin=%d, Cout=%d, stride %d)" % (B * H * W_, Cin, Cout, stride))
@@ -518,10 +603,19 @@
     d.loader, d.epi, d.tile = L.LOAD_CONV3X3, (L.EPI_PLAIN if S == 1 else L.EPI_PARTIAL), (tile if S == 1 else 0)
     d.splitk = S if S > 1 else 0
     d.conv_H, d.conv_W, d.conv_C, d.conv_OH, d.conv_OW, d.conv_stride = H, W_, Cin, OH, OW, stride
-    _gemm_launch(d, "sp3_gemm(conv3x3)", "conv3x3")
+    global _pair
+    held, _pair = _pair, None
+    try:
+        _gemm_launch(d, "sp3_gemm(conv3x3)", "conv3x3")
+    finally:
+        _pair = held
     if S > 1:
         reduce_ln(splitk_ws, S, M, Cout, bias=bias, res=res1, ldres=Cout, x_out=out, ldx=Cout, act=act, res2=res2, ldres2=Cout)
     return out
+
+
+def conv3x3_takes_res2_up(Wp, map_dtype, B, H, W_):
+    return LEAN and isinstance(Wp, PackedWeight) and Wp.dtype == torch.bfloat16 and map_dtype == torch.bfloat16 and B * H * W_ < 2048
 
 
 def conv_splitk(M, N, K, wdtype):
```
